# rhasspy/piper

Measured on AMD Instinct MI355X. Metric: audio samples/sec, higher is better.
Workload: dtype f32; 1 GPU; BASELINE configs[1]: medium VITS voice (22050 Hz), 1 utterance(s) x 128 phoneme ids per step per GPU, scales 0.667/1.0/0.8; step = inferSeconds span: host ids in (pe_upload) + pe_run, engine draws both noise sites + int16 PCM to host (pe_fetch); parallelism=utterance-parallel x1, one process per GPU, RCCL weight broadcast

## Files before the change

piper_amd/csrc/engine.h:

```cpp
#pragma once
#include <cstdint>
#include <deque>
#include <list>
#include <map>
#include <string>
#include <unordered_map>
#include <vector>

#include "pe_rt.h"
#include "engine_buffers.h"
#include "kernels/params.h"
#include "policy.h"
#include "weights.h"

namespace pe {

struct PackedConv {
  float* wp = nullptr;
  float* wp16 = nullptr;
  float* wpb = nullptr;
  const float* wunscale = nullptr;
  float* wpg4 = nullptr;
  float* bias = nullptr;
  int rows = 0;
// ... 84 lines not shown
  int native_rate() const { return rs_native_ ? rs_native_ : arch_[A_SR]; }
  int output_rate() const { return rs_on_ ? rs_out_ : native_rate(); }
  int resample_half_width() const { return rs_on_ ? rs_K_ : 0; }
  int64_t out_samples(int64_t s) const { return rs_on_ ? (s * rs_L_ + rs_M_ - 1) / rs_M_ : s; }
  void debug_resample(const float* x, int batch, int64_t stride, const int32_t* vlen, const int64_t* n0, const int32_t* count,
                      const int64_t* origin, float* out, int64_t out_stride);

  void set_loudness(bool on, float target_lufs, float ceiling_db);
  bool loudness_on() const { return ld_on_; }
  float loudness_target() const { return ld_T_; }
  float loudness_ceiling_db() const { return ld_cdb_; }
  int last_loudness(float* lufs, float* scale, float* peak, int32_t* flags, int64_t capacity);
  static void loudness_filter(int fs, double coef[10]);
  void set_loudness_ceiling(int kind);
  int loudness_ceiling_kind() const { return ld_kind_; }
  static int true_peak_oversample(int fs) { return fs > 0 ? (192000 + fs - 1) / fs : 0; }
  int last_true_peak(float* t, int64_t capacity);
  static void true_peak_filter(int fs, int& Q, int& K, std::vector<double>& coef);
  void debug_true_peak(const float* x, int batch, int64_t stride, const int32_t* valid, int fs, float* t);
  void set_loudness_limiter(bool on, float window_ms);
  bool loudness_limiter_on() const { return lim_on_; }
  float loudness_limiter_ms() const { return lim_ms_; }
  int loudness_limiter_window() const { return output_rate() > 0 ? limiter_window_samples(output_rate(), lim_ms_) : 0; }
  int last_limiter(float* max_reduction, int32_t* shaped_samples, float* trim, int64_t capacity);
  static void limiter_window(int fs, float window_ms, int& W, std::vector<double>& coef);
  void debug_limiter(const float* x, int batch, int64_t stride, const int32_t* valid, int fs, const float* g, float ceiling_db,
                     int kind, float window_ms, float* env, int16_t* pcm);
  void debug_loudness(const float* x, int batch, int64_t stride, const int32_t* valid, int fs, float target, float ceiling_db,
                      float* lufs, float* scale, int32_t* flags);

  void set_stream_gain(int mode, float peak, int ramp_samples);
  int stream_gain_mode() const { return gain_mode_; }
  float stream_gain_peak() const { return gain_peak_; }
  int stream_gain_ramp() const { return gain_ramp_; }
  int stream_last_gains(float* gain, float* peak, int64_t capacity);

  struct StreamChunk {
    int batch = 0;
    const int64_t* sample_offsets = nullptr;
    const int16_t* pcm = nullptr;
    const float* audio = nullptr;
    const int32_t* frames_done = nullptr;
  };
  const std::vector<int32_t>& stream_begin_batch(const int64_t* ids, const int64_t* offsets, int B, const float* scales,
                                                 const int64_t* sids, const NoiseIn* noise, const TimingIn* timing = nullptr,
                                                 const SeedsIn* seeds = nullptr, const BlendIn* blend = nullptr);
  void stream_next_batch(int chunk_frames, bool want_audio, StreamChunk& out);

  int stream_pool_open(int slots, int max_frames);
  void stream_pool_join(const int64_t* ids, const int64_t* offsets, int n, const float* scales, const int64_t* sids,
                        const NoiseIn* noise, int32_t* slot_of, int32_t* total_frames, const TimingIn* timing = nullptr,
                        const SeedsIn* seeds = nullptr, const BlendIn* blend = nullptr);
  void stream_pool_next(int chunk_frames, const int32_t* per_slot, bool want_audio, StreamChunk& out);
  void stream_pool_leave(int slot);
  void stream_pool_close();
  int stream_pool_state(int32_t* frames, int32_t* frames_done, int32_t* live) const;
  void stream_pool_require() const;

  int batch() const { return B_; }
  const std::vector<int64_t>& sample_offsets() { finish_run(); return sample_off_; }
  const float* audio_host() const { return h_audio_.get(); }
  const int16_t* pcm_host() const { return pcm_zc_live_ ? h_pcm_zc_.get() : h_pcm_.get(); }
  const std::vector<int32_t>& durations_host();
  const std::vector<int32_t>& frames_host() { finish_run(); return frames_h_; }
  void debug_tensor(const std::string& name, int b, std::vector<float>& out, int* rows, int* cols);
  void debug_randn(int site, uint64_t call, int64_t row, int64_t n, float* out);
  uint64_t rng_call() const { return call_; }
  long run_launches() const { return run_launches_; }
  long speculation_runs() const { return spec_runs_; }
  long speculation_misses() const { return spec_misses_; }
  const int* xcc_pattern(int* period) const { if (period) *period = xcd_period_; return xcc_of_; }

  void set_seed(uint64_t s) { seed_ = s; }
  uint64_t seed() const { return seed_; }
  void set_use_graphs(bool on) { use_graphs_ = on; }
  void set_profile(int level);
  const std::vector<ProfileRow>& profile();
  void reset_profile();
  hipStream_t stream() const { return stream_; }
  const int32_t* arch() const { return arch_; }
  int sample_rate() const { return arch_[A_SR]; }
  int hop() const { return hop_; }
  size_t weight_bytes() const { return weight_bytes_; }

 private:
  LaunchPolicy pol_;
  void init(const WeightSet& ws);
  float* dev_copy(const std::vector<float>& v);
  float* dev_alloc(size_t nfloats, const float* src);
  char* arena_ = nullptr; size_t arena_bytes_ = 0, arena_off_ = 0;
  bool arena_owned_ = false, skeleton_ = false;
  float* dev_tensor(const WeightSet& ws, const std::string& name);
  PackedConv pack_conv(const WeightSet& ws, const std::string& wname, const std::string& bname, int dil,
                       int padl_override, bool gate, int in_rev, int out_rev);
  PackedConv pack_qkv(const WeightSet& ws, const std::string& prefix, float** out16 = nullptr);
  PackedConv pack_convT(const WeightSet& ws, const std::string& prefix, int stride);
  PackedConv pack_matrix(const std::vector<float>& W, int rows, int Cin, int ntaps,
                         const std::vector<float>* bias, int nbias, int dil, int padl, bool gate, int split);
  DdsW load_dds(const WeightSet& ws, const std::string& prefix);
  enum Fill { FILL_NONE, FILL_ZERO, FILL_POISON, FILL_POISON_OR_ZERO };
  template <class Buf>
  void side_alloc(Buf& b, size_t n, bool idle, Fill fill, const char* what = nullptr, size_t what_bytes = 0);
  void ensure_stage_a(int B, int Tmax);
  void ensure_stage_b(int Fmax, int batch = 0);

  struct View { float* p; long bs; int cs; };
  struct ConvOpt {
    float in_slope = 1.f; int act = 0; View res{nullptr, 0, 0}; View out2{nullptr, 0, 0}; int mode = 0; float alpha = 1.f;
    const float* bias2 = nullptr; int bias2_bs = 0;
  };
  void conv(const PackedConv& pc, View x, View out, const int* lens, int len_mul, int Lmax, int epi, const ConvOpt& o);
  void conv(const PackedConv& pc, View x, View out, const int* lens, int len_mul, int Lmax, int epi) { conv(pc, x, out, lens, len_mul, Lmax, epi, ConvOpt()); }
  struct ConvPlan plan_conv(const PackedConv& pc, int Lmax, int epi, bool stage_tiled) const;
  bool grouping_ = false;
  bool stage_tiled_ = false;
  bool group_tiled_ = false;
  int group_cfg_ = 0;
  std::vector<struct ConvP> group_;
  double group_flops_ = 0, group_bytes_ = 0;
  int group_ncols_ = 0;
  void group_begin(bool tiled = false);
  void group_end();
  bool can_group_sum() const;
  void group_end_sum(View out, const float* bias_sum, float alpha);
  void layer_norm(View in, View out, const float* g, const float* b, int C, const int* lens, int Lmax);
  struct DdsOpt {
    const float* pre_z = nullptr; long pre_z_bs = 0; const float* pre_w = nullptr; const float* pre_b = nullptr;
    const float* z_scale = nullptr;
    const float* post_w16 = nullptr; const float* post_bias = nullptr; int post_rows = 0;
    View post_out{nullptr, 0, 0};
    const float* zin = nullptr; long zin_bs = 0; int z_cs = 0, c0 = 0, c1 = 1; float* zout = nullptr; long zout_bs = 0;
  };
  void dds(const DdsW& d, View in, View out, View tmp, const DdsOpt* opt = nullptr);
  double dds_bytes(const struct DdsP& p) const;
  double cols_ids_ = 0, cols_frames_ = 0;
  void dds_params(const DdsW& d, View in, View out, View tmp, const DdsOpt* opt, std::vector<struct DdsP>& list);
  float* pack16(const std::vector<float>& W, int rows, int K);
  float* pack4(const std::vector<float>& W, int rows, int K);
  std::unordered_map<const float*, const float*> w4_of_;
  const float* pack_ffn1(const WeightSet& ws, const std::string& wname);
  const float* pack_ffn2(const WeightSet& ws, const std::string& wname);
  DevBuf<float> ffn_parts_;
  bool stage_a_ffn_fused() const;
  float* stage_a_enc_out() const;
  const float* w4_of(const float* w16) const { auto it = w4_of_.find(w16); return it == w4_of_.end() ? nullptr : it->second; }
  float* dp_proj16_ = nullptr;
  float* dp_pre16_ = nullptr;
  float* projpre4_ = nullptr; float* projpre_bias_ = nullptr; int projpre_split_ = 0;
  void colchain(const struct ColP& p, int B, int Lmax, double flops);
  bool conv1x1_col4(const float* w16, const float* bias, int rows, View in, View out, const int* lens, int B, int Lmax,
                    double flops, const float* bias2 = nullptr, long bias2_bs = 0, const float* w4direct = nullptr, int kin = 192,
                    long max_cols = 0);
  const float* pack4_conv_pad192(const WeightSet& ws, const std::string& wname, int in_rev, int out_rev);
  struct LnSecond { const float* w4 = nullptr; int split = 0; View out2{nullptr, 0, 0}; const float* bias2 = nullptr; long bias2_bs = 0; };
  void lngemm(View y, const float* g, const float* b, View x, const float* w16, const float* bias, int rows, View out,
              int T, double flops, const float* parts = nullptr, int nparts = 0, const float* pbias = nullptr,
              const LnSecond* second = nullptr);
  bool proj_pre_stacked() const;
  float* pack16_conv(const WeightSet& ws, const std::string& wname, int in_rev, int out_rev);
  int xcc_of_[64] = {0};
  int xcd_period_ = 0;
  void probe_xcds();
  static size_t col4_smem() { return ((size_t)4 * 196 + 4 * 192 * 4 + 32 + 64 * 4) * sizeof(float); }
  void issue_stage_a();
  void issue_stage_b();
  void issue_flow();
  void issue_window();
  void issue_decoder(const float* zsrc, const int* lens, int Fmax, double fsum, bool zero_absmax, bool with_pcm16 = true,
                     const float* cond = nullptr, int cond_bs = 0);
  void run_stage(char which, const std::string& key);
  void dispatch_stage(char which);
  void drop_graphs();
  bool finish_run();
  void finish_stage_b_sizes();
  bool spec_pending_ = false;
  int spec_fg_ = 0;
  int spec_fg_force_ = 0;
  float last_ratio_ = 0.f, spec_margin_ = 1.10f;
  long spec_misses_ = 0, spec_runs_ = 0;
  int spec_hit_streak_ = 0, spec_recent_misses_ = 0, spec_recent_runs_ = 0, spec_cooldown_ = 0;
  int* d_framesc_ = nullptr;
  const int* lens_b_ = nullptr;
  void prof_begin();
  void prof_end(int row, double flops);

  int32_t arch_[ARCH_INTS];
  int device_ = 0;
  hipStream_t stream_ = nullptr;
  int H_, C_, FC_, nh_, dk_, nlayers_, ksz_, window_, hop_, U_;
  std::vector<void*> owned_;
  size_t weight_bytes_ = 0;

  float* emb_ = nullptr;
  float* emb_g_ = nullptr;
  struct EncLayer {
    PackedConv qkv, o, f1, f2;
    float* o16 = nullptr;
    float* qkv16 = nullptr;
    const float *f1p = nullptr, *f2p = nullptr;
    float *relk, *relv, *g1, *b1, *g2, *b2;
  };
  std::vector<EncLayer> enc_;
  PackedConv enc_proj_;
  float* enc_proj16_ = nullptr;
  PackedConv dp_pre_, dp_proj_;
  DdsW dp_dds_;
  struct CFlow {
    float *pre_w, *pre_b;
    DdsW dds;
    PackedConv proj;
    float* proj16 = nullptr;
  };
  std::vector<CFlow> cflows_;
  float ea_m0_ = 0, ea_es0_ = 1;
  float *ea_dev_m_ = nullptr, *ea_dev_logs_ = nullptr;
 public:
  void arena_ready();
 private:
  struct Rcl {
    PackedConv pre, post;
    float *pre16 = nullptr, *post16 = nullptr;
    const float* pre4pad = nullptr;
    std::vector<PackedConv> in, rs;
    std::vector<const float*> rs4;
    int in_off, out_off;
  };
  std::vector<Rcl> rcls_;
  PackedConv dec_pre_;
  struct UpStage {
    PackedConv up;
    int rate, ch;
    std::vector<std::vector<PackedConv>> rb;
    float* last_bias_sum = nullptr;
    struct HostConv { std::vector<float> w; int co = 0, ci = 0, k = 0, dil = 1; const float* bias = nullptr; };
    std::vector<std::vector<HostConv>> rb_host;
    void* mrf_phases = nullptr; float* mrf_w = nullptr;
    float* mrf_wsplit = nullptr; float* mrf_unscale = nullptr; int mrf_wsplit_floats = 0;
    int mrf_wfloats = 0, mrf_cp = 0, mrf_hx = 0;
    std::vector<struct MrfPhase> mrf_ph;
    bool mrf_ok = false, mrf_rb1 = false;
  };
  struct MrfGeo { int ou = 0, N = 0, cu_lo = 0, cu_hi = 0, nleft = 0, nhalo = 0; };
  bool mrf_geo(const UpStage& st, int len_mul, bool tail, MrfGeo& best) const;
  void build_mrf(UpStage& st);
  void mrf(const UpStage& st, View x, View out, const int* lens, int len_mul, int Lmax, bool tail = false);
  enum StageForm { STAGE_FUSED, STAGE_GROUP_SPLITK, STAGE_GROUP_TILED, STAGE_CHAIN };
  struct StageSchedule { StageForm form; bool tiled; };
  StageSchedule stage_schedule(const UpStage& st, int Lmax, double fsum, bool buffers_fit) const;
  bool matrix_bf3_ = false, pack_bf3_now_ = false;
  int matrix_sm_ = 0;
  static bool env_bf3();
 public:
  bool matrix_bf3() const { return matrix_bf3_; }
  int matrix_split_mode() const { return matrix_bf3_ ? matrix_sm_ : -1; }
 private:
  std::vector<UpStage> ups_;
  float* post_w_ = nullptr;
  int post_cin_ = 0;
  struct CondW { float* w; float* b; int rows; };
  CondW cond_dp_{nullptr, nullptr, 0}, cond_dec_{nullptr, nullptr, 0};
  std::vector<CondW> cond_wn_;
  int gin_ = 0, nspk_ = 1;

  int B_ = 0, Tmax_ = 0, Ts_ = 0, Fmax_ = 0, Fs_ = 0, Tg_ = 0, Fg_ = 0;
  bool use_graphs_ = true;
  struct GraphEntry { std::string key; void* exec; long launches; };
  std::list<GraphEntry> graphs_;
  std::unordered_map<std::string, std::list<GraphEntry>::iterator> graph_of_;
  long graph_captures_ = 0;
 public:
  long graph_captures() const { return graph_captures_; }
  size_t graphs_cached() const { return graphs_.size(); }
  static int id_bucket(int T);
  static int frame_bucket(int F);
  void warmup(int max_batch, int max_ids, float frames_per_id, const float* scales, const int64_t* sample, int64_t n_sample);
 private:
  long run_launches_ = 0;
  unsigned long long* d_rng_ = nullptr;
  float scales_[3] = {0.667f, 1.0f, 0.8f};
  std::vector<float> spec_rel_;
  float spec_rel(int b) const { return (size_t)b < spec_rel_.size() ? spec_rel_[b] : 1.f; }
  bool have_noise_w_ = false, have_noise_z_ = false;
  bool drew_w_ = false;
  bool plan_on_ = false, plan_skip_ = false;
  int* d_plan_ = nullptr; float* plan_w_ = nullptr;
  PinBuf<int> h_plan_;
  static bool check_timing(const TimingIn& t, const int64_t* offsets, int B);
  void plan_params(PlanP& pp, const DurP& dp) const;
  std::string stage_a_key(int B) const;
  bool fold_dur_ = false;
  DurP fold_dp_{};
  std::vector<int64_t> id_off_;
  std::vector<int32_t> tlens_h_, frames_h_, dur_h_;
  std::vector<int64_t> sample_off_;
  uint64_t seed_ = 1234, call_ = 0;
  const float* h_noise_z_ = nullptr;
  int64_t h_noise_z_stride_ = 0;

  size_t capA_B_ = 0, capA_T_ = 0, capB_B_ = 0, capB_F_ = 0;
  bool capB_exact_ = false;
  size_t ws_budget_ = 0;
  size_t ws_budget();
  DevBuf<char> wsA_, wsB_;
  int *d_ids_ = nullptr, *d_tlens_ = nullptr, *d_sids_ = nullptr, *d_dur_ = nullptr, *d_cum_ = nullptr,
      *d_frames_ = nullptr;
  float* d_scales_ = nullptr;
  static size_t in_scale_slots(size_t Bc) { return (3 * Bc + 3) & ~(size_t)3; }
  static size_t in_seed_bytes(size_t Bc) { return (12 * Bc + 15) & ~(size_t)15; }
  static size_t in_head_bytes(size_t Bc) { return 32 + in_seed_bytes(Bc); }
  unsigned long long* d_keys_ = nullptr; int* d_use_ = nullptr;
  bool seeded_ = false;
  const char* seed_key() const { return seeded_ ? "|s" : ""; }
  char* d_in_ = nullptr; PinBuf<char> h_in_; size_t in_bytes_ = 0;
  size_t in_blend_bytes(size_t Bc) const { return nspk_ > 1 ? (Bc * (68 + 4 * (size_t)gin_) + 255) & ~(size_t)255 : 0; }
  char* h_in() const { return h_in_.get() + in_blend_bytes(capA_B_); }
  char* d_blend_ = nullptr;
  float* g_tab_ = nullptr; int* g_rows_ = nullptr;
  bool blended_ = false;
  const char* blend_key() const { return blended_ ? "|g" : ""; }
  BlendP blend_params(const char* area, size_t Bc) const;
  bool ids_zc_ = false;
  unsigned long long upload_serial_ = 0;
  float* att_s_ = nullptr;
  size_t attn_smem(int T, bool global_scores) const;
  bool attn_scores_global(int T) const;
  float* vQ_ = nullptr;
  float* kT_ = nullptr;
  bool kt_on_ = false, kt_valid_ = false;
  float *x_ = nullptr, *y_ = nullptr, *qkv_ = nullptr, *att_ = nullptr, *ffh_ = nullptr, *stats_ = nullptr,
        *xg_ = nullptr, *dh_ = nullptr, *dy_ = nullptr, *dy2_ = nullptr, *hproj_ = nullptr, *z2_ = nullptr,
        *logw_ = nullptr, *noise_w_ = nullptr, *cond_ = nullptr;
  int cond_bs_ = 0;
  std::vector<int> cond_off_wn_;
  int cond_off_dp_ = 0, cond_off_dec_ = 0;
  float *zp_ = nullptr, *fh_ = nullptr, *facts_ = nullptr, *fskip_ = nullptr, *noise_z_ = nullptr;
  float* hb_[5] = {nullptr, nullptr, nullptr, nullptr, nullptr};
  hipStream_t ls_ = nullptr;
  DevBuf<float> side_[9];
  size_t side_floats_ = 0;
  float* zwin_ = nullptr;
  int* d_win_ = nullptr;
  int halo_frames_ = 0, s_frames_ = 0, s_pos_ = 0, s_wg_ = 0;
  bool s_active_ = false;
  std::vector<int16_t> s_pcm_;
  struct ChunkRows {
    char stage;
    int cap = 0;
    PinBuf<int> host; DevBuf<int> dev;
    PinBuf<int> gctl; DevBuf<int> gdev;
    std::vector<char> gfirst;
    std::vector<int32_t> pos;
    std::vector<int64_t> off;
    PinBuf<int16_t> pcm; PinBuf<float> audio;
    int wg = 0;
    const float* src = nullptr; long src_bs = 0; int src_cs = 0;
    const float* cond = nullptr; int cond_bs = 0;
  };
  void rows_free(ChunkRows& r);
  bool rows_next(ChunkRows& r, const int32_t* frames, const int32_t* live, int chunk, const int32_t* per_row, int clamp,
                 bool want_audio, StreamChunk& out);
  void issue_window_rows(const ChunkRows& r);
  bool sb_active_ = false;
  ChunkRows batch_rows_{'V'};
  void ensure_stream_batch(int B);
  int gain_mode_ = GAIN_CHUNK, gain_ramp_ = 0;
  float gain_peak_ = 0.f;
  float s_gain_r_ = 0.01f; bool s_gain_first_ = true;
  void gain_blocks_alloc(ChunkRows& r, int cap);
  void gain_prepare(int* ctl, int cap, const std::vector<char>& first, int n);
  void gain_collect(const int* ctl, int cap, int n, std::vector<char>& first, const int64_t* off, const unsigned* peaks);
  void gain_report_idle(const int* ctl, int cap, int n);
  std::vector<float> lg_gain_, lg_peak_;
  std::vector<char> lg_got_;
  int lg_n_ = -1;
  const unsigned* lg_dev_peaks_ = nullptr;
  bool lg_lazy_ = false;
  void stream_front(int B, int max_frames);
// ... 105 lines not shown
```

piper_amd/csrc/engine_issue.cpp:

```cpp
#include "engine_internal.h"

namespace pe {

bool Engine::stage_a_ffn_fused() const {
  double tsum = 0;
  for (int b = 0; b < B_; ++b) tsum += tlens_h_[b];
  const bool chain_q = pol_.chain16(tsum, false, H_, 96);
  bool f = pol_.ffn && chain_q && pol_.chain4((long)B_ * Tg_) && ffn_parts_ && (long)B_ * rup(Tg_, 4) <= LaunchPolicy::ffn_max_cols &&
           FC_ % 48 == 0 && FC_ / 48 <= 16 && w4_of(enc_proj16_);
  for (auto& e : enc_) f = f && e.f1p && e.f2p && w4_of(e.qkv16);
  return f;
}
bool Engine::proj_pre_stacked() const {
  double tsum = 0;
  for (int b = 0; b < B_; ++b) tsum += tlens_h_[b];
  return pol_.stack_pre && projpre4_ && projpre_split_ == enc_proj_.rows && dp_pre_.rows == 192 && H_ == 192 &&
         pol_.chain16(tsum, false, H_, 96) && pol_.chain4((long)B_ * Tg_);
}
float* Engine::stage_a_enc_out() const { return (stage_a_ffn_fused() && (enc_.size() & 1)) ? y_ : x_; }

void Engine::issue_stage_a() {
  const int B = B_, Ts = Ts_, T = Tg_;
  const long bsH = (long)H_ * Ts;
  auto V = [&](float* p, int ch) { return View{p, (long)ch * Ts, Ts}; };
// ... 134 lines not shown
    } else {
      conv(e.o, att, y, d_tlens_, 1, T, EPI_RESADD, {.res = x});
    }
    if (!chain_o) layer_norm(y, x, e.g1, e.b1, H_, d_tlens_, T);
    }
    if (ffn_fused) {
      FfnP fp{};
      fp.xcd = pol_.xcd_ffn ? xcd_period_ : 0;
      const int Tp = rup(T, 4);
      fp.x = x.p; fp.x_bs = x.bs; fp.x_cs = x.cs;
      fp.w1p = e.f1p; fp.b1 = e.f1.bias; fp.w2p = e.f2p;
      fp.parts = ffn_parts_.get(); fp.nslices = nsl; fp.p_bs = (long)nsl * H_ * Tp;
      fp.lens = d_tlens_;
      const int khf = kbegin(prof_level_ >= 2 ? krow("ffn_kernel") : 0, 2.0 * tsum * (e.f1.macs_per_col + e.f2.macs_per_col),
                             4.0 * (tsum * (1.0 + nsl) * H_ + e.f1.macs_per_col + e.f2.macs_per_col));
      const size_t smemf = ((size_t)192 * 48 + 4 * 48 * 16 + 48 * 48) * sizeof(float);
      launch::ffn(dim3((T + 11) / 12, nsl, B), smemf, stream_, fp);
      kend(khf);
      pend_bias = e.f2.bias;
    } else {
      conv(e.f1, x, ffh, d_tlens_, 1, T, EPI_STORE, {.act = ACT_RELU});
      conv(e.f2, ffh, y, d_tlens_, 1, T, EPI_RESADD, {.res = x});
    }
    if (chain_q) { pg = e.g2; pb = e.b2; }
    else layer_norm(y, x, e.g2, e.b2, H_, d_tlens_, T);
    fl += 2.0 * tsum * (e.qkv.macs_per_col + e.o.macs_per_col + e.f1.macs_per_col + e.f2.macs_per_col);
    for (int b = 0; b < B; ++b) fl += 2.0 * 2.0 * (double)tlens_h_[b] * tlens_h_[b] * H_;
  }
  const bool stacked = pg && proj_pre_stacked();
  LnSecond sec;
  if (stacked) {
    sec.w4 = projpre4_; sec.split = projpre_split_; sec.out2 = dy;
    sec.bias2 = cb_dp; sec.bias2_bs = cond_bs_;
  }
  const float* pj_bias = stacked ? projpre_bias_ : enc_proj_.bias;
  const int pj_rows = stacked ? projpre_split_ + dp_pre_.rows : enc_proj_.rows;
  const double pj_flops = 2.0 * tsum * (enc_proj_.macs_per_col + (stacked ? dp_pre_.macs_per_col : 0));
  if (pg && pend_bias) {
    lngemm(x, pg, pb, y, enc_proj16_, pj_bias, pj_rows, stats, T, pj_flops, ffn_parts_.get(), nsl, pend_bias, stacked ? &sec : nullptr);
    std::swap(x, y);
  } else if (pg) lngemm(y, pg, pb, x, enc_proj16_, pj_bias, pj_rows, stats, T, pj_flops, nullptr, 0, nullptr, stacked ? &sec : nullptr);
  else conv(enc_proj_, x, stats, d_tlens_, 1, T, EPI_STORE);
  if (x.p != stage_a_enc_out()) throw std::runtime_error("internal: encoder output buffer bookkeeping");
  fl += 2.0 * tsum * enc_proj_.macs_per_col;
  prof_end(0, fl);

  prof_begin();
  fl = 0;
  if (plan_skip_) {
    DurP dp{};
    dp.scales = d_scales_; dp.lens = d_tlens_; dp.dur = d_dur_; dp.cum = d_cum_; dp.d_bs = Ts; dp.frames = d_frames_;
    dp.frames_host = h_frames_.get(); dp.frames_clamped = d_framesc_; dp.frame_cap = std::max(Fs_, 1);
    PlanP pp{};
    plan_params(pp, dp);
    PE_LAUNCH_KB("duration_plan_kernel", 4.0 * 4.0 * tsum, launch::duration_plan(dim3(B), stream_, pp));
    prof_end(1, fl);
    return;
  }
  if (!stacked &&
      !(chain_q && dp_pre16_ && conv1x1_col4(dp_pre16_, dp_pre_.bias, dp_pre_.rows, x, dy, d_tlens_, B, T, 2.0 * tsum * dp_pre_.macs_per_col,
                                             cb_dp, cond_bs_)))
    conv(dp_pre_, x, dy, d_tlens_, 1, T, EPI_STORE, {.bias2 = cb_dp, .bias2_bs = cond_bs_});
  if (pol_.fuse_dp) {
    DdsOpt o;
    o.post_w16 = dp_proj16_; o.post_bias = dp_proj_.bias; o.post_rows = dp_proj_.rows; o.post_out = xg;
    dds(dp_dds_, dy, dh, dy2, &o);
  } else {
    dds(dp_dds_, dy, dh, dy2);
    conv(dp_proj_, dh, xg, d_tlens_, 1, T, EPI_STORE);
  }
  fl += 2.0 * tsum * (2 + arch_[A_DDSLAYERS]) * dp_pre_.macs_per_col;
  if (!have_noise_w_ && !drew_w_)
    PE_LAUNCH_KB("randn_kernel", 4.0 * 2.0 * tsum, launch::randn(stream_, noise_w_, (long)B * 2, T, (long)Ts, 0L, d_rng_, 0,
                                                               seeded_ ? d_keys_ : nullptr, d_use_, 2));
  if (!pol_.fuse_dp) {
    const long n = (long)B * 2 * Ts;
    PE_LAUNCH_K("scale_kernel", launch::scale(dim3((unsigned)((n + 255) / 256)), stream_, noise_w_, z2_, n, d_scales_ + 2, (long)2 * Ts));
  }
  int flips = 0;
  for (size_t fi = 0; fi < cflows_.size(); ++fi) {
    auto& cf = cflows_[fi];
    ++flips;
    const int c0 = (flips & 1) ? 1 : 0;
    const int c1 = 1 - c0;
    if (pol_.fuse_dp) {
      const float* zin = fi == 0 ? noise_w_ : z2_;
      DdsOpt o;
      o.pre_z = zin + (long)c0 * Ts; o.pre_z_bs = (long)2 * Ts; o.pre_w = cf.pre_w; o.pre_b = cf.pre_b;
      o.z_scale = fi == 0 ? d_scales_ + 2 : nullptr;
      o.post_w16 = cf.proj16; o.post_bias = cf.proj.bias; o.post_rows = cf.proj.rows;
      o.zin = zin; o.zin_bs = (long)2 * Ts; o.z_cs = Ts; o.c0 = c0; o.c1 = c1; o.zout = z2_; o.zout_bs = (long)2 * Ts;
      dds(cf.dds, xg, dh, dy2, &o);
    } else {
      PE_LAUNCH_K("cf_pre_kernel", launch::cf_pre(dim3((T + 63) / 64, H_, B), stream_, z2_ + (long)c0 * Ts, (long)2 * Ts, cf.pre_w, cf.pre_b, xg_, (long)H_ * Ts, Ts, dy_, (long)H_ * Ts, Ts, d_tlens_, H_));
      dds(cf.dds, dy, dh, dy2);
      conv(cf.proj, dh, hproj, d_tlens_, 1, T, EPI_STORE);
      PE_LAUNCH_K("spline_inverse_kernel", launch::spline_inverse(dim3((T + 63) / 64, B), stream_, hproj_, (long)32 * Ts, Ts, z2_ + (long)c1 * Ts, (long)2 * Ts, d_tlens_, 1.0f / std::sqrt((float)H_)));
    }
    fl += 2.0 * tsum * (arch_[A_DDSLAYERS] * dp_pre_.macs_per_col + cf.proj.macs_per_col);
  }
  ++flips;
  {
    const int c0 = (flips & 1) ? 1 : 0;
    DurP dp{};
    dp.z0 = z2_ + (long)c0 * Ts; dp.z_bs = (long)2 * Ts; dp.m0 = ea_m0_; dp.es0 = ea_es0_; dp.scales = d_scales_;
    dp.lens = d_tlens_; dp.dur = d_dur_; dp.cum = d_cum_; dp.d_bs = Ts; dp.frames = d_frames_; dp.logw_out = logw_;
    dp.frames_host = h_frames_.get(); dp.frames_clamped = d_framesc_; dp.frame_cap = std::max(Fs_, 1);
    fold_dp_ = dp;
    if (plan_on_) {
      PlanP pp{};
      plan_params(pp, dp);
      PE_LAUNCH_KB("duration_plan_kernel", 4.0 * 6.0 * tsum, launch::duration_plan(dim3(B), stream_, pp));
    } else if (!fold_dur_) PE_LAUNCH_KB("duration_kernel", 4.0 * 4.0 * tsum, launch::duration(dim3(B), stream_, dp));
  }
  prof_end(1, fl);
}

void Engine::issue_flow() {
  const int B = B_, Ts = Ts_, Fmax = Fg_, Fs = Fs_;
  double fsum = 0;
  for (int b = 0; b < B; ++b) fsum += frames_h_[b];
  cols_frames_ = fsum;
  double fl = 0;

  prof_begin();
  if (have_noise_z_) {
    if (h_noise_z_stride_ < Fmax_) throw std::runtime_error("noise_z stride shorter than the frame count");
    for (int b = 0; b < B; ++b)
      for (int c = 0; c < C_; ++c)
        PE_HIP(hipMemcpyAsync(noise_z_ + ((size_t)b * C_ + c) * Fs,
                              h_noise_z_ + ((size_t)b * C_ + c) * h_noise_z_stride_,
                              frames_h_[b] * sizeof(float), hipMemcpyHostToDevice, stream_));
  }
  {
    RegP rp{};
    rp.stats = stats_; rp.s_bs = (long)2 * C_ * Ts; rp.s_cs = Ts;
    rp.cum = d_cum_; rp.d_bs = Ts; rp.tlens = d_tlens_; rp.frames = lens_b_;
    rp.noise = noise_z_; rp.n_bs = (long)C_ * Fs; rp.n_cs = Fs;
    rp.scales = d_scales_;
    rp.out = zp_; rp.o_bs = (long)C_ * Fs; rp.o_cs = Fs; rp.C = C_;
    rp.absmax = absmax_;
    rp.rng = d_rng_; rp.gen = have_noise_z_ ? 0 : 1;
    if (seeded_) { rp.keys = d_keys_; rp.use = d_use_; }
    rp.fold = fold_dur_ ? 1 : 0;
    if (fold_dur_) rp.dur = fold_dp_;
    PE_LAUNCH_KB("regulate_kernel", 4.0 * (2.0 * C_ * cols_ids_ + 3.0 * C_ * fsum), launch::regulate(dim3((Fmax + 255) / 256, (C_ + 3) / 4, B), stream_, rp));
    if (zp_keep_)
      PE_HIP(hipMemcpyAsync(zp_keep_, zp_, (size_t)B * C_ * Fs * sizeof(float), hipMemcpyDeviceToDevice, stream_));
  }
  auto VF = [&](float* p, int ch) { return View{p, (long)ch * Fs, Fs}; };
  const View fh = VF(fh_, H_), facts = VF(facts_, H_), fskip = VF(fskip_, H_);
  const int half = C_ / 2;
  const bool chain = pol_.chain16(fsum, true, H_, half);
  for (size_t ri = 0; ri < rcls_.size(); ++ri) {
    Rcl& r = rcls_[ri];
    const View x0{zp_ + (long)r.in_off * Fs, (long)C_ * Fs, Fs};
    const View x1{zp_ + (long)r.out_off * Fs, (long)C_ * Fs, Fs};
    if (!(chain && ri > 0)) {
      if (!(chain && r.pre4pad && conv1x1_col4(nullptr, r.pre.bias, r.pre.rows, x0, fh, lens_b_, B, Fmax, 2.0 * fsum * r.pre.macs_per_col,
                                               nullptr, 0, r.pre4pad, half, LaunchPolicy::col4_max_frames)))
        conv(r.pre, x0, fh, lens_b_, 1, Fmax, EPI_STORE);
    }
    const int nl = (int)r.in.size();
    const bool rs_front = chain && nl >= 1 && r.rs4[nl - 1] && r.rs[nl - 1].rows == H_ && H_ == 192 && half == 96 &&
                          pol_.chain_rs_front((long)B * Fmax) && w4_of(r.post16) &&
                          (ri + 1 >= rcls_.size() || (rcls_[ri + 1].pre.rows <= 192 && w4_of(rcls_[ri + 1].pre16)));
    for (int i = 0; i < nl; ++i) {
      const float* b2 = nspk_ > 1 ? cond_ + cond_off_wn_[ri] + (long)i * 2 * H_ : nullptr;
      conv(r.in[i], fh, facts, lens_b_, 1, Fmax, EPI_GATE, {.bias2 = b2, .bias2_bs = cond_bs_});
      if (rs_front && i == nl - 1) {
        fl += 2.0 * fsum * (r.in[i].macs_per_col + r.rs[i].macs_per_col);
        continue;
      }
      if (r.rs4[i] && pol_.chain4_frames((long)B * Fmax) && H_ == 192 && r.rs[i].rows <= 2 * H_) {
        ColP cp{};
        cp.in1 = facts.p; cp.in1_bs = facts.bs; cp.in1_cs = facts.cs; cp.K1 = H_;
        cp.w1 = r.rs4[i]; cp.b1 = r.rs[i].bias; cp.rows1 = r.rs[i].rows;
        cp.mode = 2; cp.first = i == 0 ? 1 : 0;
        cp.xcd = xcd_period_;
        cp.x1 = fh.p; cp.x1_bs = fh.bs; cp.x1_cs = fh.cs;
        cp.out = fskip.p; cp.out_bs = fskip.bs; cp.out_cs = fskip.cs;
        cp.lens = lens_b_;
        const int kh4 = kbegin(prof_level_ >= 2 ? krow("colchain4_kernel<false>") : 0, 2.0 * fsum * r.rs[i].macs_per_col,
                               4.0 * (fsum * (H_ + 2.0 * cp.rows1) + (double)cp.rows1 * H_));
        launch::colchain4(dim3((Fmax + 3) / 4, B, (cp.rows1 + 191) / 192), col4_smem(), stream_, cp);
        kend(kh4);
      } else {
        conv(r.rs[i], facts, fh, lens_b_, 1, Fmax, EPI_WNRS, {.out2 = fskip, .mode = i == 0 ? 1 : 0});
      }
      fl += 2.0 * fsum * (r.in[i].macs_per_col + r.rs[i].macs_per_col);
    }
    if (chain) {
      ColP cp{};
      cp.in1 = fskip.p; cp.in1_bs = fskip.bs; cp.in1_cs = fskip.cs; cp.K1 = H_;
      cp.w1 = r.post16; cp.b1 = r.post.bias; cp.rows1 = half;
      cp.mode = 1;
      cp.x1 = x1.p; cp.x1_bs = x1.bs; cp.x1_cs = x1.cs;
      if (ri + 1 < rcls_.size()) {
        const Rcl& nx = rcls_[ri + 1];
        if (nx.in_off != r.out_off) throw std::runtime_error("coupling layers do not alternate halves");
        cp.w2 = nx.pre16; cp.b2 = nx.pre.bias; cp.rows2 = H_;
        cp.out2 = fh.p; cp.o2_bs = fh.bs; cp.o2_cs = fh.cs;
      }
      cp.lens = lens_b_;
      if (rs_front) {
        cp.in0 = facts.p; cp.in0_bs = facts.bs; cp.in0_cs = facts.cs;
        cp.w0 = r.rs4[nl - 1]; cp.b0 = r.rs[nl - 1].bias; cp.first = nl == 1 ? 1 : 0;
      }
      colchain(cp, B, Fmax, 2.0 * fsum * (r.post.macs_per_col + (cp.w2 ? rcls_[ri + 1].pre.macs_per_col : 0) +
                                          (rs_front ? r.rs[nl - 1].macs_per_col : 0)));
    } else {
      conv(r.post, fskip, x1, lens_b_, 1, Fmax, EPI_SUBFROM);
    }
    fl += 2.0 * fsum * (r.pre.macs_per_col + r.post.macs_per_col);
  }
  prof_end(2, fl);

}

void Engine::issue_stage_b() {
  issue_flow();
  double fsum = 0;
  for (int b = 0; b < B_; ++b) fsum += frames_h_[b];
  issue_decoder(zp_, lens_b_, Fg_, fsum, false);
}

void Engine::issue_window() {
  PE_LAUNCH_K("window_copy_kernel", launch::window_copy(dim3((s_wg_ + 63) / 64, C_), stream_, zp_, Fs_, d_win_, zwin_, Fs_, C_));
  issue_decoder(zwin_, d_win_ + 1, s_wg_, (double)s_wg_, true);
  if (rs_on_) issue_resample(1, audio_, Ss_, rs_host_.get(), nullptr, out_samples((long)s_wg_ * hop_) + 1, (double)s_wg_ * hop_);
}

void Engine::issue_window_rows(const ChunkRows& r) {
  const int B = (int)r.pos.size(), cap = r.cap, wg = r.wg;
  int *const dst = r.dev.get(), *const gctl = r.gctl.get(), *const gdev = r.gdev.get();
  struct Restore { int& b; int b0; ~Restore() { b = b0; } } restore{B_, B_};
  B_ = B;
  const int gm = gain_mode_;
  if (gm != GAIN_CHUNK && (!gctl || !gdev || B > cap)) throw std::runtime_error("stream gain blocks are not sized for this call");
  PE_LAUNCH_KB("window_gather_kernel", 8.0 * B * C_ * wg,
               launch::window_gather(dim3((wg + 63) / 64, C_, B), stream_, r.src, r.src_bs, r.src_cs, r.host.get(), dst, cap,
                                     noise_z_, (long)C_ * Fs_, Fs_, wg));
  std::vector<int32_t> win((size_t)B, wg);
  frames_h_.swap(win);
  try {
    issue_decoder(noise_z_, dst + sb_o_len(cap), wg, (double)B * wg, true, false, r.cond, r.cond_bs);
  } catch (...) {
    frames_h_.swap(win);
    throw;
  }
  frames_h_.swap(win);
  if (rs_on_) {
    const long max_out = out_samples((long)wg * hop_) + 1;
    issue_resample(B, audio_, Ss_, rs_host_.get(), nullptr, max_out, (double)B * wg * hop_);
    const int rsteps = std::max(1, (int)((max_out + CHUNK_SPB - 1) / CHUNK_SPB));
    if (gm != GAIN_CHUNK) {
      PE_LAUNCH_K("stream_gain_kernel", launch::stream_gain(stream_, gctl, gdev, cap, B, gm, dst, hop_, rs_dev_.get(), rs_cap_, So_));
      PE_LAUNCH_KB("chunk_pcm_rs_gain_kernel", 10.0 * B * (double)max_out,
                   launch::chunk_pcm_rs_gain(dim3(rsteps, B), stream_, raudio_.get(), So_, rs_dev_.get(), rs_cap_, dst, cap, gdev));
      return;
    }
    PE_LAUNCH_KB("chunk_pcm_rs_kernel", 10.0 * B * (double)max_out,
                 launch::chunk_pcm_rs(dim3(rsteps, B), stream_, raudio_.get(), So_, rs_dev_.get(), rs_cap_, dst, cap));
    return;
  }
  const int steps = std::max(1, (int)(((long)wg * hop_ + CHUNK_SPB - 1) / CHUNK_SPB));
  if (gm != GAIN_FIXED)
    PE_LAUNCH_KB("chunk_peak_kernel", 4.0 * B * wg * hop_, launch::chunk_peak(dim3(steps, B), stream_, audio_, Ss_, dst, cap, hop_));
  if (gm != GAIN_CHUNK) {
    PE_LAUNCH_K("stream_gain_kernel", launch::stream_gain(stream_, gctl, gdev, cap, B, gm, dst, hop_, nullptr, 0, 0));
    PE_LAUNCH_KB("chunk_pcm_gain_kernel", 10.0 * B * wg * hop_,
                 launch::chunk_pcm_gain(dim3(steps, B), stream_, audio_, Ss_, dst, cap, hop_, gdev));
    return;
  }
  PE_LAUNCH_KB("chunk_pcm_kernel", 10.0 * B * wg * hop_, launch::chunk_pcm(dim3(steps, B), stream_, audio_, Ss_, dst, cap, hop_));
}

void Engine::issue_decoder(const float* zsrc, const int* lens, int Fmax, double fsum, bool zero_absmax, bool with_pcm16,
                           const float* cond, int cond_bs) {
  const int B = B_, Fs = Fs_;
  const float* cb_dec = nspk_ > 1 ? (cond ? cond : cond_ + cond_off_dec_) : nullptr;
  const int cb_dec_bs = cond ? cond_bs : cond_bs_;
  double fl = 0;
  bool tail_done = false;
  if (zero_absmax) PE_HIP(hipMemsetAsync(absmax_, 0, B * sizeof(unsigned), stream_));
  prof_begin();
  fl = 0;
  {
    View cur{hb_[0], (long)U_ * Fs, Fs};
    conv(dec_pre_, View{const_cast<float*>(zsrc), (long)C_ * Fs, Fs}, cur, lens, 1, Fmax, EPI_STORE, {.bias2 = cb_dec, .bias2_bs = cb_dec_bs});
    fl += 2.0 * fsum * dec_pre_.macs_per_col;
    int mult = 1;
    int cur_buf = 0;
    const int nk = arch_[A_NRB];
    const float inv_nk = 1.0f / (float)nk;
    for (auto& st : ups_) {
      int ids[5], n = 0;
      for (int i = 0; i < 5 && n < 4; ++i)
        if (i != cur_buf) ids[n++] = i;
      const int Lin = mult;
      mult *= st.rate;
      const long Ls = (long)Fs * mult;
      auto VS = [&](int bi) { return View{hb_[bi], (long)st.ch * Ls, (int)Ls}; };
      const View u = VS(ids[0]), ta = VS(ids[1]), tb = VS(ids[2]), tc = VS(ids[3]);
      const int Lmax = Fmax * mult;
      const StageSchedule sched = stage_schedule(st, Lmax, fsum, (size_t)B * st.ch * Ls <= side_floats_);
      const bool fuse = sched.form == STAGE_FUSED, grp_t = sched.form == STAGE_GROUP_TILED;
      const bool tail = fuse && pol_.mrf_tail && &st == &ups_.back() && st.mrf_cp == 32 && st.ch == post_cin_ && mult == hop_;
      conv(st.up, cur, u, lens, Lin, Fmax * Lin, EPI_CONVT, {.in_slope = 0.1f});
      fl += 2.0 * fsum * Lin * st.up.macs_per_col;
      struct Scope { bool& f; ~Scope() { f = false; } } scope{stage_tiled_};
      stage_tiled_ = sched.tiled;
      const View xs{hb_[cur_buf], (long)st.ch * Ls, (int)Ls};
      auto chain = [&](int j, const View (&t)[3], View dst, int accmode) {
        auto& cv = st.rb[j];
        const int last_epi = EPI_ACCUM;
        View xin = u;
        if (arch_[A_RESBLOCK] == 1) {
          const int np = (int)cv.size() / 2;
          for (int d = 0; d < np; ++d) {
            conv(cv[2 * d], xin, t[0], lens, mult, Lmax, EPI_STORE, {.in_slope = 0.1f});
            if (d < np - 1) {
              const View nxt = (d & 1) ? t[2] : t[1];
              conv(cv[2 * d + 1], t[0], nxt, lens, mult, Lmax, EPI_RESADD, {.in_slope = 0.1f, .res = xin});
              xin = nxt;
            } else {
              conv(cv[2 * d + 1], t[0], dst, lens, mult, Lmax, last_epi, {.in_slope = 0.1f, .res = xin, .mode = accmode, .alpha = inv_nk});
            }
            fl += 2.0 * fsum * mult * (cv[2 * d].macs_per_col + cv[2 * d + 1].macs_per_col);
          }
        } else {
          const int nc = (int)cv.size();
          for (int d = 0; d < nc; ++d) {
            if (d < nc - 1) {
              const View nxt = (d & 1) ? t[2] : t[1];
              conv(cv[d], xin, nxt, lens, mult, Lmax, EPI_RESADD, {.in_slope = 0.1f, .res = xin});
              xin = nxt;
            } else {
              conv(cv[d], xin, dst, lens, mult, Lmax, last_epi, {.in_slope = 0.1f, .res = xin, .mode = accmode, .alpha = inv_nk});
            }
            fl += 2.0 * fsum * mult * cv[d].macs_per_col;
          }
        }
      };
      if (fuse) {
        mrf(st, u, xs, lens, mult, Lmax, tail);
        for (auto& cv : st.rb)
          for (auto& c : cv) fl += 2.0 * fsum * mult * c.macs_per_col;
        if (tail) {
          tail_done = true;
          fl += 2.0 * fsum * hop_ * post_cin_ * POST_K;
// ... 67 lines not shown
```

piper_amd/csrc/engine_launch.cpp:

```cpp
#include "engine_internal.h"

namespace pe {


static int tile_cfg_of(int cfg) { return cfg == CFG_C ? CFG_C : CFG_S; }
static int slab_halo(int xhalo) { return xhalo <= 64 ? 64 : 128; }
static size_t tile_smem(int nbuf, int BN, int halo) { return (size_t)nbuf * KC * ((BN + halo + 63) / 64 * 64) * sizeof(float); }
static size_t splitk_smem(int nw, int MT, int xw) { return std::max<size_t>((size_t)nw * KC * xw, (size_t)nw * MT * 16 * 64) * sizeof(float); }

ConvPlan Engine::plan_conv(const PackedConv& pc, int Lmax, int epi, bool stage_tiled) const {
  ConvPlan pl;
  const bool convt = epi == EPI_CONVT;
  const int ncols = pl.ncols = convt ? Lmax + 1 : Lmax;
  const int xhalo = (pc.ntaps - 1) * pc.dil, units = pc.nchunks * pc.ntaps;
  pl.blocks = tile_workgroups(CFG_BM[pc.cfg], CFG_BN[pc.cfg], ncols, pc.mtiles, B_);
  pl.halo = slab_halo(xhalo);
  const bool to_splitk = !stage_tiled && pol_.splitk(pl.blocks, xhalo, pc.Cin);
  const bool direct = pol_.one_tap_direct(pc.gate, convt, pc.ntaps, pc.Cin);
  pl.group_splitk = !stage_tiled && !convt && pol_.groupable(pc.gate, pc.up != 0, pl.blocks, xhalo, pc.Cin);
  pl.group_tiled = !pc.gate && pc.up == 0 && !convt && !to_splitk && !(matrix_bf3_ && pc.wpb) && !direct && xhalo <= 128;
  pl.group_cfg = tile_cfg_of(pc.cfg);
  if (to_splitk && epi == EPI_GATE &&
      pol_.gate_12col(pc.gate, pc.wpg4 != nullptr && pc.Cin == 192, pc.ntaps, pc.dil, tile_workgroups(32, 12, ncols, pc.split / 32, B_))) {
    pl.form = CONV_GATE12;
// ... 92 lines not shown
    if (cv.size() != st.rb[0].size()) grp = grp_t = false;
    for (auto& c : cv) {
      const ConvPlan pl = plan_conv(c, Lmax, EPI_STORE, tiled);
      grp = grp && pl.group_splitk;
      grp_t = grp_t && pl.group_tiled && pl.group_cfg == tc;
    }
  }
  return {grp ? STAGE_GROUP_SPLITK : (grp_t ? STAGE_GROUP_TILED : STAGE_CHAIN), tiled};
}

void Engine::group_begin(bool tiled) {
  grouping_ = true;
  group_tiled_ = tiled;
  group_cfg_ = -1;
  group_.clear();
  group_flops_ = group_bytes_ = 0;
}
void Engine::group_end() {
  grouping_ = false;
  if (group_.empty()) return;
  if (group_tiled_) {
    group_tiled_ = false;
    std::stable_sort(group_.begin(), group_.end(), [](const ConvP& a, const ConvP& b) { return a.ntaps > b.ntaps; });
    ConvG g{};
    int n = 0, rows = 0, xhalo = 0;
    for (const ConvP& c : group_) {
      g.c[n++] = c;
      rows = std::max(rows, c.rows);
      xhalo = std::max(xhalo, c.xhalo);
    }
    g.n = n;
    g.B = B_;
    const int cfg = group_cfg_, BM = CFG_BM[cfg], BN = CFG_BN[cfg];
    const int HALO = slab_halo(xhalo);
    const dim3 grid((group_ncols_ + BN - 1) / BN, (rows + BM - 1) / BM, n * B_);
    int kh = -1;
    if (prof_level_ >= 2) {
      char nm[96];
      snprintf(nm, sizeof(nm), "conv_mfma_group_kernel<%s,%d>", cfg == CFG_C ? "1,4,1,1,16" : "2,2,1,1,16", HALO);
      kh = kbegin(krow(std::string(nm)), group_flops_, group_bytes_);
    }
    launch::conv_tile_group(cfg, HALO, grid, tile_smem(2, BN, HALO), ls_, g);
    kend(kh);
    group_.clear();
    return;
  }
  constexpr int NW = 4;
  std::stable_sort(group_.begin(), group_.end(), [](const ConvP& a, const ConvP& b) { return a.ntaps > b.ntaps; });
  for (int wide = 0; wide < 2; ++wide) {
    ConvG g{};
    int n = 0, mt = 0;
    for (const ConvP& c : group_)
      if ((c.xhalo > 32) == (wide == 1)) {
        g.c[n++] = c;
        mt = std::max(mt, (c.rows + 31) / 32);
      }
    if (!n) continue;
    g.n = n;
    g.B = B_;
    const dim3 grid((group_ncols_ + 31) / 32, mt, n * B_);
    const double share = (double)n / (double)group_.size();
    const int kh = kbegin(prof_level_ >= 2 ? krow(wide ? "conv_splitk_group_kernel<4,2,128>" : "conv_splitk_group_kernel<4,2,64>") : 0,
                          group_flops_ * share, group_bytes_ * share);
    launch::conv_group(wide != 0, grid, splitk_smem(NW, 1, wide ? 128 : 64), ls_, g);
    kend(kh);
  }
  group_.clear();
}

bool Engine::can_group_sum() const {
  if (group_.size() < 2 || group_.size() > 3) return false;
  const ConvP& a = group_[0];
  for (const ConvP& c : group_)
    if (c.rows != a.rows || c.Cin != a.Cin || c.nchunks != a.nchunks || c.x_bs != a.x_bs || c.x_cs != a.x_cs ||
        c.r_bs != a.r_bs || c.r_cs != a.r_cs || c.in_slope != a.in_slope || c.epi != EPI_RESADD || c.xhalo > 96)
      return false;
  return true;
}
void Engine::group_end_sum(View out, const float* bias_sum, float alpha) {
  grouping_ = false;
  if (!can_group_sum()) throw std::runtime_error("internal: convs do not fit a K-concatenated launch");
  ConvP q = group_[0];
  q.nseg = (int)group_.size();
  for (int i = 0; i < q.nseg; ++i) {
    q.seg_x[i] = group_[i].x; q.seg_wp[i] = group_[i].wp;
    q.seg_ntaps[i] = group_[i].ntaps; q.seg_dil[i] = group_[i].dil; q.seg_padl[i] = group_[i].padl;
  }
  q.res2 = group_[1].res;
  q.res3 = q.nseg > 2 ? group_[2].res : nullptr;
  q.bias = bias_sum;
  q.out = out.p; q.o_bs = out.bs; q.o_cs = out.cs;
  q.epi = EPI_ACCUM; q.mode = 3; q.alpha = alpha;
  q.tgroups = 1;
  const dim3 grid((group_ncols_ + 31) / 32, (q.rows + 31) / 32, B_);
  const int kh = kbegin(prof_level_ >= 2 ? krow("conv_splitk_sum_kernel<4,2>") : 0, group_flops_, group_bytes_);
  launch::conv_group_sum(grid, splitk_smem(4, 1, 128), ls_, q);
  kend(kh);
  group_.clear();
}

static void conv_cost(const PackedConv& pc, int epi, int mode, double cols, double& flops, double& bytes) {
  const bool rd_res = epi == EPI_RESADD || epi == EPI_ACCUM;
  const bool rd_old = epi == EPI_SUBFROM || epi == EPI_WNRS || (epi == EPI_ACCUM && (mode == 1 || mode == 2));
  const double out_rows = epi == EPI_GATE ? pc.split : pc.rows;
  flops = 2.0 * pc.macs_per_col * cols;
  bytes = 4.0 * (cols * (pc.Cin + out_rows * (1 + (rd_res ? 1 : 0) + (rd_old ? 1 : 0))) + (double)pc.rows * pc.Cin * pc.ntaps);
}

void Engine::conv(const PackedConv& pc, View x, View out, const int* lens, int len_mul, int Lmax, int epi, const ConvOpt& o) {
  if ((epi == EPI_GATE) != pc.gate) throw std::runtime_error("internal: gate epilogue/packing mismatch");
  ConvP p;
  p.x = x.p; p.x_bs = x.bs; p.x_cs = x.cs;
  p.wp = pc.wp; p.wp16 = pc.wp16; p.wpb = pc.wpb; p.wunscale = pc.wunscale; p.wpg4 = nullptr; p.bias = pc.bias;
  p.bias2 = o.bias2; p.bias2_bs = o.bias2_bs;
  p.out = out.p; p.o_bs = out.bs; p.o_cs = out.cs;
  p.res = o.res.p; p.r_bs = o.res.bs; p.r_cs = o.res.cs;
  p.out2 = o.out2.p; p.o2_bs = o.out2.bs; p.o2_cs = o.out2.cs;
  p.lens = lens; p.len_mul = len_mul;
  p.Cin = pc.Cin; p.rows = pc.rows; p.nchunks = pc.nchunks;
  p.ntaps = pc.ntaps; p.dil = pc.dil; p.padl = pc.padl; p.xhalo = (pc.ntaps - 1) * pc.dil;
  p.in_slope = o.in_slope; p.epi = epi; p.act = o.act; p.mode = o.mode; p.alpha = o.alpha;
  p.split = (epi == EPI_GATE) ? pc.split : (epi == EPI_WNRS ? (pc.rows > H_ ? H_ : 0) : 0);
  p.up = pc.up; p.padT = pc.padT; p.up_magic = pc.up ? (unsigned)((0x100000000ULL + pc.up - 1) / pc.up) : 0u;
  p.up_vec = 0; p.tpb = 1; p.tgroups = 1;
  double kflops = 0, kbytes = 0;
  if (prof_level_ >= 2) {
    const std::vector<int32_t>& lh = (lens == d_tlens_) ? tlens_h_ : frames_h_;
    double cols = 0;
    for (int b = 0; b < B_; ++b) cols += (double)lh[b] * len_mul;
    conv_cost(pc, epi, o.mode, cols, kflops, kbytes);
  }
  const ConvPlan pl = plan_conv(pc, Lmax, epi, stage_tiled_);
  if (grouping_) {
    if (!(group_tiled_ ? pl.group_tiled : pl.group_splitk) || group_.size() >= 3 ||
        (!group_.empty() && (group_ncols_ != pl.ncols || (group_tiled_ && group_cfg_ != pl.group_cfg))))
      throw std::runtime_error(group_tiled_ ? "internal: conv does not fit a grouped tiled launch" : "internal: conv does not fit a grouped launch");
    group_cfg_ = pl.group_cfg;
    group_.push_back(p);
    group_ncols_ = pl.ncols;
    group_flops_ += kflops; group_bytes_ += kbytes;
    return;
  }
  p.up_vec = pl.up_vec; p.tpb = pl.tpb; p.tgroups = pl.tgroups;
  if (pl.form == CONV_GATE12) p.wpg4 = pc.wpg4;
  const int kh = prof_level_ >= 2 ? kbegin(krow(conv_row_name(pl, pc, matrix_sm_, pol_.prof_sites != 0, epi, len_mul)), kflops, kbytes) : -1;
  switch (pl.form) {
    case CONV_GATE12: launch::gate4(pl.grid, pl.smem, ls_, p); break;
    case CONV_SPLITK: launch::conv_splitk(pc.gate, pl.nw, pl.grid, pl.smem, ls_, p); break;
    case CONV_SPLITK16: launch::conv_splitk16(pc.gate, pl.grid, pl.smem, ls_, p, pl.half); break;
    case CONV_SPLIT: launch::conv_bf3(matrix_sm_, pl.cfg, pc.gate, pl.halo, pl.grid, pl.smem, ls_, p); break;
    case CONV_1X1: launch::conv1x1(pl.grid, ls_, p); break;
    case CONV_TILE: launch::conv_tile(pl.cfg, pc.gate, pl.halo, pl.grid, pl.smem, ls_, p); break;
  }
  kend(kh);
}

bool Engine::mrf_geo(const UpStage& st, int len_mul, bool tail, MrfGeo& best) const {
  const int CP = st.mrf_cp, NCG = CP == 32 ? 8 : 4, HU = CP == 32 ? 1 : 2;
  const int OUMAX = CP == 32 ? 4 : 3;
  const int hx = st.mrf_hx, hxa = rup(hx, 16);
  auto geo = [&](int ou, MrfGeo& g) {
    g.ou = ou; g.N = 16 * NCG * ou;
    if (hxa + g.N + hx > mrf_ws(CP, ou)) return false;
    g.cu_lo = (hxa - hx) / 16; g.cu_hi = (hxa + g.N + hx + 15) / 16;
    g.nleft = hxa / 16 - g.cu_lo; g.nhalo = g.cu_hi - g.cu_lo - g.N / 16;
    return g.nhalo <= NCG * HU;
  };
  best = MrfGeo{};
  double best_cost = 0;
  MrfGeo forced;
  const int force = (pol_.mrf_ou >= 1 && pol_.mrf_ou <= OUMAX && geo((int)pol_.mrf_ou, forced)) ? (int)pol_.mrf_ou : 0;
  for (int ou = 1; ou <= OUMAX; ++ou) {
    MrfGeo g;
    if ((force && ou != force) || !geo(ou, g)) continue;
    double wgs = 0;
    const int stride = tail ? g.N - (POST_K - 1) : g.N;
    for (int b = 0; b < B_; ++b) wgs += (double)(((long)frames_h_[b] * len_mul + stride - 1) / stride);
    double work = 0, taps = 0;
    for (auto& P : st.mrf_ph) {
      const int lo = (hxa - P.e) / 16, hi = (hxa + g.N + P.e + 15) / 16;
      work += (double)(hi - lo) * 16 * P.ntaps;
      taps += P.ntaps;
    }
    double cost = std::ceil(wgs / 256.0) * (work + 16.0 * taps);
    if (ou == 4) cost *= 1.06;
    if (!best.ou || cost < best_cost) { best = g; best_cost = cost; }
  }
  return best.ou != 0;
}

void Engine::mrf(const UpStage& st, View x, View out, const int* lens, int len_mul, int Lmax, bool tail) {
  const int CP = st.mrf_cp, HU = CP == 32 ? 1 : 2;
  const int hx = st.mrf_hx, hxa = rup(hx, 16);
  MrfGeo best;
  if (!mrf_geo(st, len_mul, tail, best)) throw std::runtime_error("internal: no mrf_kernel geometry for this stage");
  MrfP p{};
  p.x = x.p; p.x_bs = x.bs; p.x_cs = x.cs;
  p.out = out.p; p.o_bs = out.bs; p.o_cs = out.cs;
  p.lens = lens; p.len_mul = len_mul;
  p.phases = static_cast<const MrfPhase*>(st.mrf_phases); p.nphases = (int)st.mrf_ph.size();
  p.wstream = st.mrf_w; p.wfloats = st.mrf_wfloats;
  p.C = st.ch; p.N = best.N; p.wcols = hxa + best.N + hx; p.hxa = hxa; p.cu_lo = best.cu_lo; p.cu_hi = best.cu_hi;
  p.nleft = best.nleft; p.nhalo = best.nhalo;
  p.slope = 0.1f;
  p.alpha = 1.0f / (float)st.rb.size();
  p.stride = best.N; p.n0off = 0;
  p.post_w = nullptr; p.audio = nullptr; p.a_bs = 0; p.absmax = nullptr; p.post_slope = 0.01f;
  if (tail) {
    p.stride = best.N - (POST_K - 1); p.n0off = (POST_K - 1) / 2;
    p.post_w = post_w_; p.audio = audio_; p.a_bs = Ss_; p.absmax = absmax_;
  }
  double kflops = 0, kbytes = 0;
  if (prof_level_ >= 2) {
    double cols = 0;
    for (int b = 0; b < B_; ++b) cols += (double)frames_h_[b] * len_mul;
    double macs = 0;
    for (auto& cv : st.rb)
      for (auto& c : cv) macs += c.macs_per_col;
    kflops = 2.0 * macs * cols;
    kbytes = 8.0 * st.ch * cols + 4.0 * st.mrf_wfloats;
    if (tail) {
      kflops += 2.0 * cols * st.ch * POST_K;
      kbytes = 4.0 * (st.ch + 1) * cols + 4.0 * st.mrf_wfloats;
    }
  }
  dim3 grid((Lmax + p.stride - 1) / p.stride, B_);
  char nm[64];
  const bool split = matrix_bf3_ && pol_.mrf_split && st.mrf_wsplit != nullptr && matrix_sm_ < 2;
  if (split) {
    p.wstream = st.mrf_wsplit; p.wfloats = st.mrf_wsplit_floats; p.wunscale = st.mrf_unscale;
    snprintf(nm, sizeof(nm), "mrf_split_kernel<%d,%d,%d,%d>", matrix_sm_, CP, best.ou, HU);
  } else {
    snprintf(nm, sizeof(nm), "mrf_kernel<%d,%d,%d>", CP, best.ou, HU);
  }
  const int kh = prof_level_ >= 2 ? kbegin(krow(std::string(nm)), kflops, kbytes) : -1;
  if (split) launch::mrf_split(matrix_sm_, CP, best.ou, grid, ls_, p);
  else launch::mrf(CP, best.ou, grid, ls_, p);
  kend(kh);
}

size_t Engine::attn_smem(int T, bool global_scores) const {
  const int SP = rup(T, 64) + 1, VS = dk_ + 1 + (dk_ & 1);
  return ((global_scores ? 0 : (size_t)ATT_QB * SP) + (size_t)ATT_KCH * VS + (size_t)dk_ * ATT_QB +
          (size_t)2 * (2 * window_ + 1) * dk_ + 4 * ATT_QB * 16) * sizeof(float);
}
bool Engine::attn_scores_global(int T) const { return pol_.attn_long || attn_smem(T, false) > (size_t)160 * 1024; }

void Engine::layer_norm(View in, View out, const float* g, const float* b, int C, const int* lens, int Lmax) {
  LnP p;
  p.in = in.p; p.i_bs = in.bs; p.i_cs = in.cs;
  p.out = out.p; p.o_bs = out.bs; p.o_cs = out.cs;
  p.gamma = g; p.beta = b;
  p.lens = lens; p.C = C;
  if (C > LN_COLS * 32) throw std::runtime_error("LayerNorm over more than 256 channels is not supported");
  dim3 grid((Lmax + LN_COLS - 1) / LN_COLS, B_);
  const int kh = kbegin(prof_level_ >= 2 ? krow("ln_kernel") : 0, 0.0, 4.0 * 2.0 * C * (lens == d_tlens_ ? cols_ids_ : cols_frames_));
  launch::layer_norm(grid, stream_, p);
  kend(kh);
}

void Engine::dds_params(const DdsW& d, View in, View out, View tmp, const DdsOpt* opt, std::vector<DdsP>& list) {
  int dil = 1;
  const int n = (int)d.c1x1.size();
  View cur = in;
  for (int i = 0; i < n; ++i) {
    const View dst = ((n - 1 - i) & 1) ? tmp : out;
    if (dst.p == cur.p) throw std::runtime_error("internal: DDSConv buffer aliasing");
    DdsP p{};
    if (opt && i == 0 && opt->pre_z) {
      p.pre_z = opt->pre_z; p.pre_z_bs = opt->pre_z_bs; p.pre_w = opt->pre_w; p.pre_b = opt->pre_b;
    }
    p.z_scale = opt ? opt->z_scale : nullptr;
    if (opt && i == n - 1 && opt->post_w16) {
      p.post_w16 = opt->post_w16; p.post_w4 = w4_of(opt->post_w16); p.post_bias = opt->post_bias; p.post_rows = opt->post_rows;
      p.post_out = opt->post_out.p; p.po_bs = opt->post_out.bs; p.po_cs = opt->post_out.cs;
      p.zin = opt->zin; p.zin_bs = opt->zin_bs; p.z_cs = opt->z_cs; p.c0 = opt->c0; p.c1 = opt->c1;
      p.zout = opt->zout; p.zout_bs = opt->zout_bs;
      p.inv_sqrt_h = 1.0f / std::sqrt((float)H_);
    }
    p.x = cur.p; p.x_bs = cur.bs; p.x_cs = cur.cs;
    p.out = dst.p; p.o_bs = dst.bs; p.o_cs = dst.cs;
    p.dw_w = d.dw_w[i]; p.dw_b = d.dw_b[i]; p.dw_k = ksz_; p.dw_dil = dil;
    p.g1 = d.g1[i]; p.b1 = d.b1[i]; p.g2 = d.g2[i]; p.b2 = d.b2[i];
    p.bias = d.c1x1[i].bias;
    p.wp16 = d.w16[i];
    p.wp4 = w4_of(d.w16[i]);
    p.nchunks = d.c1x1[i].nchunks;
    p.lens = d_tlens_; p.H = H_;
    list.push_back(p);
    dil *= ksz_;
    cur = dst;
  }
}

double Engine::dds_bytes(const DdsP& p) const {
  return 4.0 * (cols_ids_ * (2.0 * H_ + p.post_rows) + (double)H_ * H_ + (double)p.post_rows * H_);
}

void Engine::dds(const DdsW& d, View in, View out, View tmp, const DdsOpt* opt) {
  std::vector<DdsP> list;
  dds_params(d, in, out, tmp, opt, list);
  bool four = H_ == 192 && ksz_ <= 3 && pol_.chain4((long)B_ * Tg_);
  for (const DdsP& p : list) four = four && p.wp4 && (!p.post_w16 || p.post_w4);
  for (const DdsP& p : list) {
    if (four) {
      const int kh4 = kbegin(prof_level_ >= 2 ? krow("dds_layer4_kernel") : 0, 0.0, dds_bytes(p));
// ... 168 lines not shown
```

piper_amd/csrc/engine_pack.cpp:

```cpp
#include "engine_internal.h"
#include <cmath>

namespace pe {


float* Engine::dev_alloc(size_t nfloats, const float* src) {
  arena_off_ = (arena_off_ + 255) / 256 * 256;
  const size_t bytes = std::max<size_t>(nfloats, 1) * sizeof(float);
  if (arena_off_ + bytes > arena_bytes_) throw std::runtime_error("internal: packed weights exceed the arena bound");
  float* d = reinterpret_cast<float*>(arena_ + arena_off_);
  arena_off_ += bytes;
  if (src && nfloats && !skeleton_) PE_HIP(hipMemcpy(d, src, nfloats * sizeof(float), hipMemcpyHostToDevice));
  weight_bytes_ += nfloats * sizeof(float);
  return d;
}
float* Engine::dev_copy(const std::vector<float>& v) { return dev_alloc(v.size(), v.data()); }

float* Engine::dev_tensor(const WeightSet& ws, const std::string& name) {
  const HostTensor& t = ws.get(name);
  return dev_alloc((size_t)t.numel(), t.data.empty() ? nullptr : t.data.data());
}

size_t Engine::arena_bound(const WeightSet& ws) {
  size_t n = 0;
// ... 159 lines not shown
  if (w.dims.size() != 3) throw std::runtime_error(wname + ": expected a rank-3 conv weight");
  const int Co = (int)w.dims[0], Ci = (int)w.dims[1], K = (int)w.dims[2];
  std::vector<float> W(skeleton_ ? 0 : (size_t)Co * Ci * K);
  if (!skeleton_) {
    if (w.data.size() != W.size()) throw std::runtime_error(wname + ": data size mismatch");
    for (int o = 0; o < Co; ++o)
      for (int i = 0; i < Ci; ++i)
        for (int k = 0; k < K; ++k) {
          const int so = out_rev ? Co - 1 - o : o, si = in_rev ? Ci - 1 - i : i;
          W[((size_t)o * Ci + i) * K + k] = w.data[((size_t)so * Ci + si) * K + k];
        }
  }
  std::vector<float> bias;
  bool has_b = !bname.empty() && ws.has(bname);
  if (has_b) {
    if (ws.get(bname).numel() != Co) throw std::runtime_error(bname + ": bias size mismatch");
    if (!skeleton_) {
      bias = ws.get(bname).data;
      if (out_rev) std::reverse(bias.begin(), bias.end());
    }
  }
  const int padl = padl_override >= 0 ? padl_override : (K - 1) * dil / 2;
  return pack_matrix(W, Co, Ci, K, has_b ? &bias : nullptr, Co, dil, padl, gate, gate ? Co / 2 : 0);
}

PackedConv Engine::pack_qkv(const WeightSet& ws, const std::string& prefix, float** out16) {
  std::vector<float> W, bias;
  int H = 0;
  for (const char* n : {"conv_q", "conv_k", "conv_v"}) {
    const HostTensor& w = ws.get(prefix + "." + n + ".weight");
    const HostTensor& b = ws.get(prefix + "." + n + ".bias");
    H = (int)w.dims[0];
    if (!skeleton_) {
      W.insert(W.end(), w.data.begin(), w.data.end());
      bias.insert(bias.end(), b.data.begin(), b.data.end());
    }
  }
  if (out16) *out16 = pack16(W, 3 * H, H);
  return pack_matrix(W, 3 * H, H, 1, &bias, 3 * H, 1, 0, false, 0);
}

PackedConv Engine::pack_convT(const WeightSet& ws, const std::string& prefix, int stride) {
  const HostTensor& w = ws.get(prefix + ".weight");
  const int Ci = (int)w.dims[0], Co = (int)w.dims[1], K = (int)w.dims[2];
  if (K != 2 * stride || ((K - stride) & 1))
    throw std::runtime_error(prefix + ": ConvTranspose1d with kernel != 2*stride is not supported");
  const int rows = Co * stride;
  std::vector<float> W(skeleton_ ? 0 : (size_t)rows * Ci * 2);
  for (int co = 0; co < (skeleton_ ? 0 : Co); ++co)
    for (int ph = 0; ph < stride; ++ph)
      for (int ci = 0; ci < Ci; ++ci) {
        const size_t row = (size_t)co * stride + ph;
        W[(row * Ci + ci) * 2 + 0] = w.data[((size_t)ci * Co + co) * K + ph + stride];
        W[(row * Ci + ci) * 2 + 1] = w.data[((size_t)ci * Co + co) * K + ph];
      }
  std::vector<float> bias = ws.get(prefix + ".bias").data;
  PackedConv pc = pack_matrix(W, rows, Ci, 2, &bias, Co, 1, 1, false, 0);
  pc.up = stride;
  pc.padT = (K - stride) / 2;
  return pc;
}

float* Engine::pack16(const std::vector<float>& W, int rows, int K) {
  const int Kp = rup(K, 32), nq = Kp / 16, ntile = (rows + 15) / 16;
  const size_t np = (size_t)ntile * nq * 256;
  std::vector<float> P(skeleton_ ? 0 : np, 0.f);
  for (int mt = 0; mt < (skeleton_ ? 0 : ntile); ++mt)
    for (int q = 0; q < nq; ++q)
      for (int lane = 0; lane < 64; ++lane)
        for (int jj = 0; jj < 4; ++jj) {
          const int row = mt * 16 + (lane & 15), ci = 4 * (4 * q + jj) + (lane >> 4);
          if (row < rows && ci < K) P[(((size_t)mt * nq + q) * 64 + lane) * 4 + jj] = W[(size_t)row * K + ci];
        }
  float* d16 = dev_alloc(np, skeleton_ ? nullptr : P.data());
  if (const float* d4 = pack4(W, rows, K)) w4_of_[d16] = d4;
  return d16;
}

float* Engine::pack4(const std::vector<float>& W, int rows, int K) {
  if (K != 192 && K != 96) return nullptr;
  const int nq = K / 4, ntile = (rows + 63) / 64;
  const size_t np = (size_t)ntile * nq * 256;
  std::vector<float> P(skeleton_ ? 0 : np, 0.f);
  for (int mt = 0; mt < (skeleton_ ? 0 : ntile); ++mt)
    for (int q = 0; q < nq; ++q)
      for (int lane = 0; lane < 64; ++lane)
        for (int jj = 0; jj < 4; ++jj) {
          const int row = mt * 64 + lane;
          if (row < rows) P[(((size_t)mt * nq + q) * 64 + lane) * 4 + jj] = W[(size_t)row * K + 4 * q + jj];
        }
  return dev_alloc(np, skeleton_ ? nullptr : P.data());
}

const float* Engine::pack_ffn1(const WeightSet& ws, const std::string& wname) {
  const HostTensor& w = ws.get(wname);
  if (w.dims.size() != 3 || w.dims[1] != 192 || w.dims[2] != 3 || w.dims[0] % 48 || w.dims[0] / 48 > 16) return nullptr;
  const int FC = (int)w.dims[0], S = FC / 48;
  const size_t np = (size_t)FC * 192 * 3;
  std::vector<float> P(skeleton_ ? 0 : np, 0.f);
  for (int s = 0; s < (skeleton_ ? 0 : S); ++s)
    for (int m = 0; m < 3; ++m)
      for (int wv = 0; wv < 4; ++wv)
        for (int tp = 0; tp < 3; ++tp)
          for (int q = 0; q < 3; ++q)
            for (int lane = 0; lane < 64; ++lane)
              for (int j = 0; j < 4; ++j) {
                const int row = 48 * s + 16 * m + (lane & 15), ch = 48 * wv + 4 * (4 * q + j) + (lane >> 4);
                P[(((((size_t)(s * 3 + m) * 4 + wv) * 3 + tp) * 3 + q) * 64 + lane) * 4 + j] = w.data[((size_t)row * 192 + ch) * 3 + tp];
              }
  return dev_alloc(np, skeleton_ ? nullptr : P.data());
}
const float* Engine::pack_ffn2(const WeightSet& ws, const std::string& wname) {
  const HostTensor& w = ws.get(wname);
  if (w.dims.size() != 3 || w.dims[0] != 192 || w.dims[2] != 3 || w.dims[1] % 48 || w.dims[1] / 48 > 16) return nullptr;
  const int FC = (int)w.dims[1], S = FC / 48;
  const size_t np = (size_t)FC * 192 * 3;
  std::vector<float> P(skeleton_ ? 0 : np, 0.f);
  for (int s = 0; s < (skeleton_ ? 0 : S); ++s)
    for (int rt = 0; rt < 12; ++rt)
      for (int tp = 0; tp < 3; ++tp)
        for (int q = 0; q < 3; ++q)
          for (int lane = 0; lane < 64; ++lane)
            for (int j = 0; j < 4; ++j) {
              const int row = 16 * rt + (lane & 15), hid = 48 * s + 4 * (4 * q + j) + (lane >> 4);
              P[((((size_t)(s * 12 + rt) * 3 + tp) * 3 + q) * 64 + lane) * 4 + j] = w.data[((size_t)row * FC + hid) * 3 + tp];
            }
  return dev_alloc(np, skeleton_ ? nullptr : P.data());
}

float* Engine::pack16_conv(const WeightSet& ws, const std::string& wname, int in_rev, int out_rev) {
  const HostTensor& w = ws.get(wname);
  if (w.dims.size() != 3 || w.dims[2] != 1) throw std::runtime_error(wname + ": expected a 1x1 conv weight");
  const int Co = (int)w.dims[0], Ci = (int)w.dims[1];
  std::vector<float> W(skeleton_ ? 0 : (size_t)Co * Ci);
  if (!skeleton_)
    for (int o = 0; o < Co; ++o)
      for (int i = 0; i < Ci; ++i)
        W[(size_t)o * Ci + i] = w.data[(size_t)(out_rev ? Co - 1 - o : o) * Ci + (in_rev ? Ci - 1 - i : i)];
  return pack16(W, Co, Ci);
}

const float* Engine::pack4_conv_pad192(const WeightSet& ws, const std::string& wname, int in_rev, int out_rev) {
  const HostTensor& w = ws.get(wname);
  if (w.dims.size() != 3 || w.dims[2] != 1 || w.dims[1] > 192) return nullptr;
  const int Co = (int)w.dims[0], Ci = (int)w.dims[1];
  std::vector<float> W(skeleton_ ? 0 : (size_t)Co * 192, 0.f);
  if (!skeleton_)
    for (int o = 0; o < Co; ++o)
      for (int i = 0; i < Ci; ++i)
        W[(size_t)o * 192 + i] = w.data[(size_t)(out_rev ? Co - 1 - o : o) * Ci + (in_rev ? Ci - 1 - i : i)];
  return pack4(W, Co, 192);
}

DdsW Engine::load_dds(const WeightSet& ws, const std::string& p) {
  DdsW d;
  for (int i = 0; i < arch_[A_DDSLAYERS]; ++i) {
    const std::string s = std::to_string(i);
    d.dw_w.push_back(dev_tensor(ws, p + ".convs_sep." + s + ".weight"));
    d.dw_b.push_back(dev_tensor(ws, p + ".convs_sep." + s + ".bias"));
    d.c1x1.push_back(pack_conv(ws, p + ".convs_1x1." + s + ".weight", p + ".convs_1x1." + s + ".bias", 1, -1,
                               false, 0, 0));
    {
      const HostTensor& w1 = ws.get(p + ".convs_1x1." + s + ".weight");
      d.w16.push_back(pack16(w1.data, (int)w1.dims[0], (int)w1.dims[1]));
    }
    d.g1.push_back(dev_tensor(ws, p + ".norms_1." + s + ".gamma"));
    d.b1.push_back(dev_tensor(ws, p + ".norms_1." + s + ".beta"));
    d.g2.push_back(dev_tensor(ws, p + ".norms_2." + s + ".gamma"));
    d.b2.push_back(dev_tensor(ws, p + ".norms_2." + s + ".beta"));
  }
  return d;
}

void Engine::init(const WeightSet& ws) {
  pol_.read_env();
  use_graphs_ = !pol_.no_graph;
  matrix_bf3_ = env_bf3();
  matrix_sm_ = std::max(0, LaunchPolicy::matrix_mode_env());
  memcpy(arch_, ws.arch, sizeof(arch_));
  PE_HIP(hipSetDevice(device_));
  PE_HIP(hipStreamCreateWithFlags(&stream_, hipStreamNonBlocking));
  ls_ = stream_;
  H_ = arch_[A_HIDDEN]; C_ = arch_[A_INTER]; FC_ = arch_[A_FILTER]; nh_ = arch_[A_NHEADS];
  nlayers_ = arch_[A_NLAYERS]; ksz_ = arch_[A_KSIZE]; window_ = arch_[A_WINDOW]; U_ = arch_[A_UPINIT];
  gin_ = arch_[A_GIN]; nspk_ = arch_[A_NSPK];
  if (H_ <= 0 || C_ <= 0 || nh_ <= 0 || H_ % nh_ || (C_ & 1)) throw std::runtime_error("bad architecture header");
  dk_ = H_ / nh_;
  if (dk_ > 128 || (dk_ & 1)) throw std::runtime_error("head dimension must be even and <= 128");
  if ((2 * window_ + 1) * dk_ > 1280 || window_ > 4)
    throw std::runtime_error("relative-attention window too wide (window <= 4, (2*window+1) * head dim <= 1280)");
  if (H_ % 32 || H_ > 256) throw std::runtime_error("hidden_channels must be a multiple of 32 and <= 256");
  if (ksz_ > 3 || !(ksz_ & 1)) throw std::runtime_error("kernel_size must be 1 or 3");
  hop_ = 1;
  for (int i = 0; i < arch_[A_NUPS]; ++i) hop_ *= arch_[A_UPR0 + i];

  emb_ = dev_tensor(ws, "enc_p.emb.weight");
  const int padl_ffn = (ksz_ - 1) / 2;
  for (int l = 0; l < nlayers_; ++l) {
    const std::string s = std::to_string(l), a = "enc_p.encoder.attn_layers." + s,
                      f = "enc_p.encoder.ffn_layers." + s;
    EncLayer e;
    e.qkv = pack_qkv(ws, a, &e.qkv16);
    e.o = pack_conv(ws, a + ".conv_o.weight", a + ".conv_o.bias", 1, -1, false, 0, 0);
    e.o16 = pack16_conv(ws, a + ".conv_o.weight", 0, 0);
    e.relk = dev_tensor(ws, a + ".emb_rel_k");
    e.relv = dev_tensor(ws, a + ".emb_rel_v");
    e.g1 = dev_tensor(ws, "enc_p.encoder.norm_layers_1." + s + ".gamma");
    e.b1 = dev_tensor(ws, "enc_p.encoder.norm_layers_1." + s + ".beta");
    e.f1 = pack_conv(ws, f + ".conv_1.weight", f + ".conv_1.bias", 1, padl_ffn, false, 0, 0);
    e.f2 = pack_conv(ws, f + ".conv_2.weight", f + ".conv_2.bias", 1, padl_ffn, false, 0, 0);
    if (H_ == 192 && ksz_ == 3 && padl_ffn == 1) {
      e.f1p = pack_ffn1(ws, f + ".conv_1.weight");
      e.f2p = pack_ffn2(ws, f + ".conv_2.weight");
    }
    e.g2 = dev_tensor(ws, "enc_p.encoder.norm_layers_2." + s + ".gamma");
    e.b2 = dev_tensor(ws, "enc_p.encoder.norm_layers_2." + s + ".beta");
    enc_.push_back(e);
  }
  enc_proj_ = pack_conv(ws, "enc_p.proj.weight", "enc_p.proj.bias", 1, -1, false, 0, 0);
  enc_proj16_ = pack16_conv(ws, "enc_p.proj.weight", 0, 0);

  dp_pre_ = pack_conv(ws, "dp.pre.weight", "dp.pre.bias", 1, -1, false, 0, 0);
  dp_pre16_ = (H_ == 192) ? pack16_conv(ws, "dp.pre.weight", 0, 0) : nullptr;
  projpre4_ = nullptr;
  projpre_bias_ = nullptr;
  projpre_split_ = 0;
  if (H_ == 192) {
    const HostTensor& wp = ws.get("enc_p.proj.weight");
    const HostTensor& wd = ws.get("dp.pre.weight");
    const HostTensor& bp = ws.get("enc_p.proj.bias");
    const HostTensor& bd = ws.get("dp.pre.bias");
    if (wp.dims.size() == 3 && wd.dims.size() == 3 && wp.dims[1] == 192 && wd.dims[1] == 192 && wp.dims[2] == 1 && wd.dims[2] == 1 &&
        wp.dims[0] % 192 == 0 && wd.dims[0] == 192) {
      const int rp = (int)wp.dims[0], rd = (int)wd.dims[0];
      std::vector<float> Wst(skeleton_ ? 0 : (size_t)(rp + rd) * 192), Bst(skeleton_ ? 0 : (size_t)(rp + rd));
      if (!skeleton_) {
        std::copy(wp.data.begin(), wp.data.begin() + (size_t)rp * 192, Wst.begin());
        std::copy(wd.data.begin(), wd.data.begin() + (size_t)rd * 192, Wst.begin() + (size_t)rp * 192);
        std::copy(bp.data.begin(), bp.data.begin() + rp, Bst.begin());
        std::copy(bd.data.begin(), bd.data.begin() + rd, Bst.begin() + rp);
      }
      projpre4_ = pack4(Wst, rp + rd, 192);
      projpre_bias_ = dev_alloc((size_t)(rp + rd), skeleton_ ? nullptr : Bst.data());
      projpre_split_ = rp;
    }
  }
  dp_dds_ = load_dds(ws, "dp.convs");
  dp_proj_ = pack_conv(ws, "dp.proj.weight", "dp.proj.bias", 1, -1, false, 0, 0);
  {
    const HostTensor& w = ws.get("dp.proj.weight");
    dp_proj16_ = pack16(w.data, (int)w.dims[0], (int)w.dims[1]);
  }
  for (int i = arch_[A_DPFLOWS] - 1; i >= 1; --i) {
    const std::string p = "dp.flows." + std::to_string(2 * i + 1);
    CFlow cf;
    cf.pre_w = dev_tensor(ws, p + ".pre.weight");
    cf.pre_b = dev_tensor(ws, p + ".pre.bias");
    cf.dds = load_dds(ws, p + ".convs");
    cf.proj = pack_conv(ws, p + ".proj.weight", p + ".proj.bias", 1, -1, false, 0, 0);
    if (cf.proj.rows != 3 * arch_[A_NBINS] - 1 || arch_[A_NBINS] != 10)
      throw std::runtime_error("spline with num_bins != 10 is not supported");
    {
      const HostTensor& w = ws.get(p + ".proj.weight");
      cf.proj16 = pack16(w.data, (int)w.dims[0], (int)w.dims[1]);
    }
    cflows_.push_back(cf);
  }
  {
    ea_dev_m_ = dev_tensor(ws, "dp.flows.0.m");
    ea_dev_logs_ = dev_tensor(ws, "dp.flows.0.logs");
    if (!skeleton_) {
      ea_m0_ = ws.get("dp.flows.0.m").data[0];
      ea_es0_ = std::exp(-ws.get("dp.flows.0.logs").data[0]);
    }
  }

  pack_bf3_now_ = matrix_bf3_;
  {
    const int nf = arch_[A_FLOWN], half = C_ / 2, wnl = arch_[A_WNLAYERS], wnk = arch_[A_WNK];
    int flips = 0;
    for (int f = nf - 1; f >= 0; --f) {
      ++flips;
      const bool odd = flips & 1;
      const std::string p = "flow.flows." + std::to_string(2 * f);
      Rcl r;
      r.in_off = odd ? half : 0;
      r.out_off = odd ? 0 : half;
      r.pre = pack_conv(ws, p + ".pre.weight", p + ".pre.bias", 1, -1, false, odd, 0);
      for (int i = 0; i < wnl; ++i) {
        const std::string s = std::to_string(i);
        r.in.push_back(pack_conv(ws, p + ".enc.in_layers." + s + ".weight", p + ".enc.in_layers." + s + ".bias",
                                 1, -1, true, 0, 0));
        r.rs.push_back(pack_conv(ws, p + ".enc.res_skip_layers." + s + ".weight",
                                 p + ".enc.res_skip_layers." + s + ".bias", 1, -1, false, 0, 0));
        {
          const HostTensor& wrs = ws.get(p + ".enc.res_skip_layers." + s + ".weight");
          r.rs4.push_back(wrs.dims.size() == 3 && wrs.dims[2] == 1 ? pack4(wrs.data, (int)wrs.dims[0], (int)wrs.dims[1]) : nullptr);
        }
        (void)wnk;
      }
      r.post = pack_conv(ws, p + ".post.weight", p + ".post.bias", 1, -1, false, 0, odd);
      r.pre16 = pack16_conv(ws, p + ".pre.weight", odd, 0);
      if (H_ == 192 && rcls_.empty()) r.pre4pad = pack4_conv_pad192(ws, p + ".pre.weight", odd, 0);
      r.post16 = pack16_conv(ws, p + ".post.weight", 0, odd);
      rcls_.push_back(r);
      if (gin_) {
        const HostTensor& cw = ws.get(p + ".enc.cond_layer.weight");
        cond_wn_.push_back(CondW{dev_tensor(ws, p + ".enc.cond_layer.weight"), dev_tensor(ws, p + ".enc.cond_layer.bias"),
                                 (int)cw.dims[0]});
      }
    }
    if (flips & 1) throw std::runtime_error("odd number of flow layers is not supported");
  }

  dec_pre_ = pack_conv(ws, "dec.conv_pre.weight", "dec.conv_pre.bias", 1, -1, false, 0, 0);
  {
    const int nk = arch_[A_NRB], nd = arch_[A_NDIL];
    int ch = U_;
    for (int i = 0; i < arch_[A_NUPS]; ++i) {
      UpStage st;
      st.rate = arch_[A_UPR0 + i];
      st.up = pack_convT(ws, "dec.ups." + std::to_string(i), st.rate);
      ch = U_ >> (i + 1);
      st.ch = ch;
      for (int j = 0; j < nk; ++j) {
        const std::string rb = "dec.resblocks." + std::to_string(i * nk + j);
        std::vector<PackedConv> cv;
        std::vector<UpStage::HostConv> hv;
        auto add = [&](const std::string& wn, const std::string& bn, int dil) {
          cv.push_back(pack_conv(ws, wn, bn, dil, -1, false, 0, 0));
          const HostTensor& w = ws.get(wn);
          UpStage::HostConv h;
          h.w = w.data; h.co = (int)w.dims[0]; h.ci = (int)w.dims[1]; h.k = (int)w.dims[2]; h.dil = dil;
          h.bias = cv.back().bias;
          hv.push_back(std::move(h));
        };
        for (int d = 0; d < nd; ++d) {
          const int dil = arch_[A_RBDIL0 + j * MAX_DIL + d];
          const std::string s = std::to_string(d);
          if (arch_[A_RESBLOCK] == 1) {
            add(rb + ".convs1." + s + ".weight", rb + ".convs1." + s + ".bias", dil);
            add(rb + ".convs2." + s + ".weight", rb + ".convs2." + s + ".bias", 1);
          } else {
            add(rb + ".convs." + s + ".weight", rb + ".convs." + s + ".bias", dil);
          }
        }
        st.rb.push_back(cv);
        st.rb_host.push_back(std::move(hv));
      }
      {
        std::vector<float> bs(skeleton_ ? 0 : (size_t)ch, 0.f);
        for (int j = 0; j < nk; ++j) {
          const std::string rb = "dec.resblocks." + std::to_string(i * nk + j);
          const std::string bn = rb + (arch_[A_RESBLOCK] == 1 ? ".convs2." : ".convs.") + std::to_string(nd - 1) + ".bias";
          if (!ws.has(bn) || ws.get(bn).numel() != ch) throw std::runtime_error(bn + ": bias size mismatch");
          if (!skeleton_)
            for (int c = 0; c < ch; ++c) bs[c] += ws.get(bn).data[c];
        }
        st.last_bias_sum = dev_alloc((size_t)ch, skeleton_ ? nullptr : bs.data());
      }
      build_mrf(st);
      st.rb_host.clear();
      ups_.push_back(st);
    }
    const HostTensor& pw = ws.get("dec.conv_post.weight");
    post_w_ = dev_tensor(ws, "dec.conv_post.weight");
    post_cin_ = (int)pw.dims[1];
    if ((int)pw.dims[0] != 1 || post_cin_ != ch || (int)pw.dims[2] != POST_K)
      throw std::runtime_error("dec.conv_post shape mismatch");
  }

  pack_bf3_now_ = false;
  if (nspk_ > 1) {
    if (!gin_) throw std::runtime_error("multi-speaker voice without gin_channels");
    emb_g_ = dev_tensor(ws, "emb_g.weight");
    const HostTensor& dw = ws.get("dp.cond.weight");
    cond_dp_ = CondW{dev_tensor(ws, "dp.cond.weight"), dev_tensor(ws, "dp.cond.bias"), (int)dw.dims[0]};
    const HostTensor& cw = ws.get("dec.cond.weight");
    cond_dec_ = CondW{dev_tensor(ws, "dec.cond.weight"), dev_tensor(ws, "dec.cond.bias"), (int)cw.dims[0]};
    cond_off_dp_ = 0;
    int off = cond_dp_.rows;
    for (auto& c : cond_wn_) { cond_off_wn_.push_back(off); off += c.rows; }
    cond_off_dec_ = off;
    off += cond_dec_.rows;
    cond_bs_ = off;
  }

  {
    long r = 3;
    const int nk = arch_[A_NRB], nd = arch_[A_NDIL];
    for (int i = (int)ups_.size() - 1; i >= 0; --i) {
      long widest = 0;
      for (int j = 0; j < nk; ++j) {
        const long hk = (arch_[A_RBK0 + j] - 1) / 2;
        long w = 0;
        for (int d = 0; d < nd; ++d) {
          w += hk * arch_[A_RBDIL0 + j * MAX_DIL + d];
          if (arch_[A_RESBLOCK] == 1) w += hk;
        }
        widest = std::max(widest, w);
      }
      r += widest;
      r = (r + ups_[i].rate - 1) / ups_[i].rate + 1;
    }
    halo_frames_ = (int)(r + 3);
  }
  launch::init_conv();
  launch::init_bf3();
  launch::init_front();
  launch::init_tail();
  probe_xcds();
  static const char* rows[] = {"text_encoder", "duration_predictor", "regulate+flow", "hifigan", "post+pcm"};
  for (auto n : rows) prof_.push_back(ProfileRow{n});
  PE_HIP(hipEventCreate(&ev0_));
  PE_HIP(hipEventCreate(&ev1_));
  h_frames_.grow(4096);
}

void Engine::build_mrf(UpStage& st) {
  const int ch = st.ch;
  if (!pol_.mrf_build(ch) || st.rb_host.empty()) return;
  const int CP = ch <= 32 ? 32 : 64, MS = CP / 16, NCH = CP / KC, STEPF = MS * 512;
  const bool rb1 = arch_[A_RESBLOCK] == 1;
  int hx = 0;
  for (auto& hv : st.rb_host) {
    int e = 0;
    for (auto& h : hv) e += h.dil * (h.k - 1) / 2;
    hx = std::max(hx, e);
  }
  const int hxa = rup(hx, 16);
  std::vector<MrfPhase> phases;
  std::vector<float> wstream;
  const bool split = matrix_bf3_ && matrix_sm_ < 2;
  std::vector<uint16_t> wsplit;
  std::vector<float> unscale;
  for (size_t j = 0; j < st.rb_host.size(); ++j) {
    auto& hv = st.rb_host[j];
    const int n = (int)hv.size();
    if (n == 0 || (rb1 && (n & 1))) return;
    int e = 0;
    for (auto& h : hv) {
      if (!(h.k & 1) || h.ci != ch || h.co != ch) return;
      e += h.dil * (h.k - 1) / 2;
    }
    for (int i = 0; i < n; ++i) {
      const auto& h = hv[i];
      e -= h.dil * (h.k - 1) / 2;
      MrfPhase P{};
      P.bias = h.bias; P.ntaps = h.k; P.dil = h.dil; P.e = e;
      const bool last = i == n - 1;
      if (rb1) {
        if (!(i & 1)) { P.src = 0; P.dst = 1; P.flags = 0; }
        else { P.src = 1; P.dst = last ? -1 : 0; P.flags = MRF_RES | MRF_KEEP; }
      } else {
        P.src = i == 0 ? 0 : 1; P.dst = last ? -1 : 1; P.flags = MRF_RES | MRF_KEEP;
        if (n > 2) return;
      }
// ... 86 lines not shown
```

piper_amd/csrc/kernels/col4.h:

```cpp
#pragma once
#include "dds.h"

namespace pe {

__device__ __forceinline__ int c4_tile(int bx, int nx, int P) { return pe_xcd_tile(bx, nx, P); }

constexpr int FFN_MAXS = 16;
constexpr int C4_H = 192, C4_NT = C4_H / 64;
template <int K>
struct Col4W {
  static constexpr int NQ = K / 16;
  static constexpr int KS = K + 4;
  f32x4 w[C4_NT][K / 16];
};
template <int K>
__device__ __forceinline__ void col_gemm4_fetch(Col4W<K>& W, const float* wp4, int nt, int wv, int lane) {
  constexpr int NQ = Col4W<K>::NQ, tile_floats = (K / 4) * 256;
#pragma unroll
  for (int m = 0; m < C4_NT; ++m) {
    const bool live = PE_UNIFORM(m < nt);
    const pe_rowsrc ws = pe_make_row_u(wp4 + (long)(live ? m : 0) * tile_floats, live ? tile_floats : 0);
#pragma unroll
    for (int q = 0; q < NQ; ++q) W.w[m][q] = pe_row_load4(ws, ((NQ * wv + q) * 64 + lane) * 4);
  }
  PE_SCHED_FENCE();
}
template <int K>
__device__ __forceinline__ void col_gemm4_run(const Col4W<K>& W, const float* YT, float* P, int wv, int lane) {
  constexpr int NQ = Col4W<K>::NQ, KS = Col4W<K>::KS;
  f32x4 acc[C4_NT];
#pragma unroll
  for (int m = 0; m < C4_NT; ++m)
#pragma unroll
    for (int r = 0; r < 4; ++r) acc[m][r] = 0.f;
  const float* yp = YT + (lane & 3) * KS + 4 * NQ * wv;
#pragma unroll
  for (int q = 0; q < NQ; ++q) {
    f32x4 yv;
#pragma unroll
    for (int j = 0; j < 4; ++j) yv[j] = yp[4 * q + j];
#pragma unroll
    for (int j = 0; j < 4; ++j)
#pragma unroll
      for (int m = 0; m < C4_NT; ++m) acc[m] = pe_mfma_4x4x1(W.w[m][q][j], yv[j], acc[m]);
  }
#pragma unroll
  for (int m = 0; m < C4_NT; ++m)
#pragma unroll
    for (int r = 0; r < 4; ++r) P[((wv * C4_NT + m) * 64 + 4 * (lane >> 2) + r) * 4 + (lane & 3)] = acc[m][r];
}
__device__ __forceinline__ float col_gemm4_get(const float* P, int c, int col) {
  const int o = c * 4 + col;
  return ((P[o] + P[C4_H * 4 + o]) + P[2 * C4_H * 4 + o]) + P[3 * C4_H * 4 + o];
}
__device__ __forceinline__ float pe_col_sum4(float v, float* red, int& flip, int wv, int lane, int col) {
  v += __shfl_xor(v, 4);
  v += __shfl_xor(v, 8);
  v += __shfl_xor(v, 16);
  v += __shfl_xor(v, 32);
  float* r = red + flip * 16;
  flip ^= 1;
  if (lane < 4) r[wv * 4 + col] = v;
  __syncthreads();
  return ((r[col] + r[4 + col]) + r[8 + col]) + r[12 + col];
}


template <bool FRONT>
__global__ __launch_bounds__(256) void colchain4_kernel(const int* lens, const float* in1, long in1_bs, int nx, int xcd, int mode,
                                                        int in1_cs, int K1r, int rows1, int first, int out_cs, ColP p) {
  PE_KTRACE(3);
  constexpr int NC = 4, NVT = 3, K1 = C4_H, K2 = C4_H / 2, KS1 = Col4W<K1>::KS, KS2 = Col4W<K2>::KS;
  PE_DYN_SMEM(float, sm);
  if constexpr (!FRONT) PE_STAMP(3, 0);
  p.lens = lens; p.xcd = xcd; p.mode = mode; p.in1 = in1; p.in1_bs = in1_bs; p.in1_cs = in1_cs; p.K1 = K1r; p.rows1 = rows1;
  p.first = first; p.out_cs = out_cs;
  const int b = blockIdx.y;
  int L = PE_UNIFORM(lens[b]);
  if constexpr (FRONT) PE_ENTRY_BATCH(L, p.res, p.res_bs, p.res_cs, p.gamma, p.beta, p.out, p.out_bs, p.x1, p.x1_bs, p.x1_cs, p.b1, p.w1,
                                      p.in0, p.in0_bs, p.in0_cs, p.w0, p.b0);
  else PE_ENTRY_BATCH(L, p.res, p.res_bs, p.res_cs, p.gamma, p.beta, p.out, p.out_bs, p.x1, p.x1_bs, p.x1_cs, p.b1, p.w1);
  const int t0 = c4_tile(blockIdx.x, nx, p.xcd) * NC;
  if (t0 >= L) return;
  if constexpr (!FRONT) PE_STAMP(3, 1);
  float* YT = sm;
  float* P = YT + NC * KS1;
  float* red = P + 4 * C4_H * NC;
  const int tid = threadIdx.x, col = tid & 3, rl = tid >> 2, wv = PE_UNIFORM(tid >> 6), lane = tid & 63;
  const int t = t0 + col;
  const bool ok = t < L;
  const int part = p.mode >= 2 ? (int)blockIdx.z : 0, row0 = part * C4_H;
  const int rows_here = p.rows1 - row0 < C4_H ? p.rows1 - row0 : C4_H;
  Col4W<K1> gw0;
  Col4W<K1> gw;
  auto fetch_gw = [&]() { col_gemm4_fetch<K1>(gw, p.w1 + (long)part * C4_NT * (K1 / 4) * 256, (rows_here + 63) / 64, wv, lane); };
  const bool skip_part = p.mode == 2 && (p.rows1 <= C4_H || part == 1);
  float sk[NVT];
  if constexpr (FRONT) {
    const pe_rowsrc a0 = pe_make_row(p.in0 + (long)b * p.in0_bs, K1 * p.in0_cs);
    const pe_rowsrc s0 = pe_make_row(p.in1 + (long)b * p.in1_bs, p.first ? 0 : K1 * p.in1_cs);
    const pe_rowsrc b0d = pe_make_row(p.b0 ? p.b0 : p.w0, p.b0 ? K1 : 0);
    float av[NVT], b0v[NVT];
#pragma unroll
    for (int k = 0; k < NVT; ++k) {
      const int c = rl + 64 * k;
      av[k] = pe_row_load(a0, ok ? c * p.in0_cs + t : -1);
      sk[k] = pe_row_load(s0, ok ? c * p.in1_cs + t : -1);
      b0v[k] = pe_row_load(b0d, c);
    }
    PE_SCHED_FENCE();
    col_gemm4_fetch<K1>(gw0, p.w0, C4_NT, wv, lane);
#pragma unroll
    for (int k = 0; k < NVT; ++k) YT[col * KS1 + rl + 64 * k] = av[k];
    __syncthreads();
    fetch_gw();
    col_gemm4_run<K1>(gw0, YT, P, wv, lane);
    __syncthreads();
#pragma unroll
    for (int k = 0; k < NVT; ++k) sk[k] = ok ? (col_gemm4_get(P, rl + 64 * k, col) + b0v[k]) + sk[k] : 0.f;
  }

  float ov[NVT], gg[NVT], bb[NVT], b1v[NVT];
  {
    const pe_rowsrc ind = pe_make_row(p.in1 + (long)b * p.in1_bs, p.K1 * p.in1_cs);
    const float* obp = p.mode == 0 ? p.res + (long)b * p.res_bs : (skip_part ? p.out + (long)b * p.out_bs : p.x1 + (long)b * p.x1_bs);
    const int ocs = p.mode == 0 ? p.res_cs : (skip_part ? p.out_cs : p.x1_cs);
    const pe_rowsrc od = p.mode == 3 ? pe_make_row(p.res ? p.res + (long)b * p.res_bs + row0 : p.w1, p.res ? rows_here : 0)
                                     : pe_make_row(obp, (skip_part && p.first) ? 0 : rows_here * ocs);
    const pe_rowsrc gd = pe_make_row(p.mode == 0 ? p.gamma : p.w1, p.mode == 0 ? p.rows1 : 0);
    const pe_rowsrc bd = pe_make_row(p.mode == 0 ? p.beta : p.w1, p.mode == 0 ? p.rows1 : 0);
    const pe_rowsrc b1d = pe_make_row(p.b1 ? p.b1 + row0 : p.w1, p.b1 ? rows_here : 0);
    float xin[NVT];
#pragma unroll
    for (int k = 0; k < NVT; ++k) {
      const int c = rl + 64 * k;
      xin[k] = FRONT ? sk[k] : pe_row_load(ind, ok ? c * p.in1_cs + t : -1);
      ov[k] = pe_row_load(od, (ok && c < rows_here) ? (p.mode == 3 ? c : c * ocs + t) : -1);
      gg[k] = pe_row_load(gd, c < rows_here ? c : -1);
      bb[k] = pe_row_load(bd, c < rows_here ? c : -1);
      b1v[k] = pe_row_load(b1d, c < rows_here ? c : -1);
    }
    PE_SCHED_FENCE();
    if constexpr (!FRONT) fetch_gw();
    if constexpr (!FRONT) PE_STAMP(3, 2);
#pragma unroll
    for (int k = 0; k < NVT; ++k) YT[col * KS1 + rl + 64 * k] = xin[k];
  }
  __syncthreads();
  col_gemm4_run<K1>(gw, YT, P, wv, lane);
  Col4W<K2> gw2;
  const bool second = p.mode == 1 && p.w2;
  if (second) col_gemm4_fetch<K2>(gw2, p.w2, (p.rows2 + 63) / 64, wv, lane);
  __syncthreads();

  if (p.mode >= 2) {
    if (!ok) return;
    float* tp = (skip_part || p.mode == 3) ? p.out + (long)b * p.out_bs + (p.mode == 3 ? (long)row0 * p.out_cs : 0) : p.x1 + (long)b * p.x1_bs;
    const int tcs = (skip_part || p.mode == 3) ? p.out_cs : p.x1_cs;
#pragma unroll
    for (int k = 0; k < NVT; ++k) {
      const int c = rl + 64 * k;
      if (c < rows_here) {
        const float val = (col_gemm4_get(P, c, col) + b1v[k]) + ov[k];
        tp[(long)c * tcs + t] = val;
        if (p.mode == 3 && p.kT && part == 1) p.kT[(long)b * p.kt_bs + ((long)(c >> 2) * p.out_cs + t) * 4 + (c & 3)] = val;
        if (p.mode == 3 && p.vQ && part == 2) p.vQ[(long)b * p.kt_bs + ((long)(t >> 2) * C4_H + c) * 4 + (t & 3)] = val;
      }
    }
    return;
  }
  if (p.mode == 0) {
    int red_flip = 0;
    auto col_sum = [&](float x) -> float { return pe_col_sum4(x, red, red_flip, wv, lane, col); };
    const int H = p.rows1;
    float v[NVT];
    float s = 0.f;
#pragma unroll
    for (int k = 0; k < NVT; ++k) {
      const int c = rl + 64 * k;
      v[k] = (ok && c < H) ? (col_gemm4_get(P, c, col) + b1v[k]) + ov[k] : 0.f;
      s += v[k];
    }
    const float mean = col_sum(s) / (float)H;
    float q = 0.f;
#pragma unroll
    for (int k = 0; k < NVT; ++k)
      if (rl + 64 * k < H) { const float d = v[k] - mean; q = fmaf(d, d, q); }
    const float rstd = 1.f / sqrtf(col_sum(q) / (float)H + 1e-5f);
    if (!ok) return;
    float* ob = p.out + (long)b * p.out_bs;
#pragma unroll
    for (int k = 0; k < NVT; ++k) {
      const int c = rl + 64 * k;
      if (c < H) ob[(long)c * p.out_cs + t] = (v[k] - mean) * rstd * gg[k] + bb[k];
    }
    return;
  }

  {
    float* xb = p.x1 + (long)b * p.x1_bs;
    float* YT2 = YT;
    const pe_rowsrc b2d = pe_make_row(second ? p.b2 : p.w1, (second && p.b2) ? p.rows2 : 0);
    float b2v[NVT];
#pragma unroll
    for (int k = 0; k < NVT; ++k) b2v[k] = pe_row_load(b2d, rl + 64 * k);
#pragma unroll
    for (int k = 0; k < NVT; ++k) {
      const int c = rl + 64 * k;
      if (c < K2) {
        const float xn = (ok && c < p.rows1) ? ov[k] - (col_gemm4_get(P, c, col) + b1v[k]) : 0.f;
        if (ok && c < p.rows1) xb[(long)c * p.x1_cs + t] = xn;
        YT2[col * KS2 + c] = xn;
      }
    }
    if (!second) return;
    __syncthreads();
    col_gemm4_run<K2>(gw2, YT2, P, wv, lane);
    __syncthreads();
    if (!ok) return;
    float* o2 = p.out2 + (long)b * p.o2_bs;
#pragma unroll
    for (int k = 0; k < NVT; ++k) {
      const int c = rl + 64 * k;
      if (c < p.rows2) o2[(long)c * p.o2_cs + t] = col_gemm4_get(P, c, col) + b2v[k];
    }
  }
}

__global__ __launch_bounds__(256) void lngemm4_kernel(const int* lens, int nx, int xcd, const float* in, long in_bs, int in_cs,
                                                      int rows, const float* parts, int nparts, LnGemmP p) {
  PE_KTRACE(7);
  constexpr int NC = 4, NVT = 3, H = C4_H, KS = Col4W<H>::KS;
  PE_DYN_SMEM(float, sm);
  p.lens = lens; p.xcd = xcd; p.in = in; p.in_bs = in_bs; p.in_cs = in_cs; p.rows = rows; p.parts = parts; p.nparts = nparts;
  const int b = blockIdx.y;
  int L = PE_UNIFORM(lens[b]);
  PE_ENTRY_BATCH(L, p.gamma, p.beta, p.bias, p.pbias, p.p_bs, p.w16);
  const int t0 = c4_tile(blockIdx.x, nx, p.xcd) * NC;
  if (t0 >= L) return;
  float* YT = sm;
  float* P = YT + NC * KS;
  float* red = P + 4 * H * NC;
  const int tid = threadIdx.x, col = tid & 3, rl = tid >> 2, wv = PE_UNIFORM(tid >> 6), lane = tid & 63;
  const int t = t0 + col;
  const bool ok = t < L;
  const int part = blockIdx.z, row0 = part * H;
  const int rows_here = p.rows - row0 < H ? p.rows - row0 : H;
  Col4W<H> gw;
  auto fetch_gw = [&]() { col_gemm4_fetch<H>(gw, p.w16 + (long)part * C4_NT * (H / 4) * 256, (rows_here + 63) / 64, wv, lane); };
  float v[NVT], gg[NVT], bb[NVT], cb[NVT];
  {
    const pe_rowsrc ind = pe_make_row(p.in + (long)b * p.in_bs, H * p.in_cs);
    const pe_rowsrc gd = pe_make_row(p.gamma, H), bd = pe_make_row(p.beta, H);
    const pe_rowsrc cbd = pe_make_row(p.bias ? p.bias + row0 : p.gamma, p.bias ? rows_here : 0);
#pragma unroll
    for (int k = 0; k < NVT; ++k) {
      const int c = rl + 64 * k;
      v[k] = pe_row_load(ind, ok ? c * p.in_cs + t : -1);
      gg[k] = pe_row_load(gd, c);
      bb[k] = pe_row_load(bd, c);
      cb[k] = pe_row_load(cbd, c);
    }
    if (p.parts) {
      const pe_rowsrc pbd = pe_make_row(p.pbias, H);
      float pv[NVT][FFN_MAXS];
      float pbv[NVT];
#pragma unroll
      for (int k = 0; k < NVT; ++k) {
        const int c = rl + 64 * k;
        pbv[k] = pe_row_load(pbd, c);
        const pe_rowsrc pd = pe_make_row(p.parts + (long)b * p.p_bs + (long)(t0 >> 2) * p.nparts * (H * 4), p.nparts * (H * 4));
#pragma unroll
        for (int sl = 0; sl < FFN_MAXS; ++sl) pv[k][sl] = pe_row_load(pd, (ok && sl < p.nparts) ? sl * (H * 4) + c * 4 + col : -1);
      }
      PE_SCHED_FENCE();
      fetch_gw();
#pragma unroll
      for (int k = 0; k < NVT; ++k) {
        float a = pv[k][0];
#pragma unroll
        for (int sl = 1; sl < FFN_MAXS; ++sl) a += pv[k][sl];
        v[k] = ok ? v[k] + (a + pbv[k]) : 0.f;
      }
    } else {
      PE_SCHED_FENCE();
      fetch_gw();
    }
  }
  int red_flip = 0;
  auto col_sum = [&](float x) -> float { return pe_col_sum4(x, red, red_flip, wv, lane, col); };
  float s = 0.f;
#pragma unroll
  for (int k = 0; k < NVT; ++k) s += v[k];
  const float mean = col_sum(s) / (float)H;
  float q = 0.f;
#pragma unroll
  for (int k = 0; k < NVT; ++k) { const float d = v[k] - mean; q = fmaf(d, d, q); }
  const float rstd = 1.f / sqrtf(col_sum(q) / (float)H + 1e-5f);
  float* xo = p.xout + (long)b * p.x_bs;
#pragma unroll
  for (int k = 0; k < NVT; ++k) {
    const int c = rl + 64 * k;
    const float y = ok ? (v[k] - mean) * rstd * gg[k] + bb[k] : 0.f;
// ... 25 lines not shown
```

piper_amd/csrc/kernels/gate4.h:

```cpp
#pragma once
#include "conv_common.h"

namespace pe {

constexpr int G4_NC = 12, G4_WC = 16, G4_NW = 12, G4_K = 192, G4_XS = G4_K + 4;
__global__ __launch_bounds__(64 * G4_NW) void gate4_kernel(const int* lens, int len_mul, const float* x, long x_bs, int x_cs,
                                                           int Cin, int padl, int ntaps_, const float* wpg4, ConvP p) {
  PE_KTRACE(4);
  PE_DYN_SMEM(float, sm);
  p.lens = lens; p.len_mul = len_mul; p.x = x; p.x_bs = x_bs; p.x_cs = x_cs; p.Cin = Cin; p.padl = padl; p.ntaps = ntaps_;
  p.wpg4 = wpg4;
  float* XT = sm;
  float* P = XT + G4_WC * G4_XS;
  const int b = blockIdx.z, grp = blockIdx.y;
  PE_STAMP(5, 0);
  const int L = p.lens[b] * p.len_mul;
  const int n0 = blockIdx.x * G4_NC;
  const int tid = threadIdx.x, lane = tid & 63, wv = PE_UNIFORM(tid >> 6);
  const int l3 = lane & 3, lb = lane >> 2;
  const int ntaps = p.ntaps;
  const pe_rowsrc xd = pe_make_row(p.x + (long)b * p.x_bs, p.Cin * p.x_cs);
  float xv[4];
#pragma unroll
  for (int u = 0; u < 4; ++u) {
    const int idx = tid + 64 * G4_NW * u, ch = idx >> 4, c = idx & 15, t = n0 - p.padl + c;
    xv[u] = pe_row_load(xd, (t >= 0 && t < p.x_cs) ? ch * p.x_cs + t : -1);
  }
  PE_SCHED_FENCE();
  f32x4 wf[5][4];
  {
    const int tap_floats = (G4_K / 4) * 256;
    const pe_rowsrc wd = pe_make_row_u(p.wpg4 + (long)grp * ntaps * tap_floats, ntaps * tap_floats);
#pragma unroll
    for (int tp = 0; tp < 5; ++tp)
#pragma unroll
      for (int q = 0; q < 4; ++q) wf[tp][q] = pe_row_load4(wd, tp < ntaps ? ((tp * (G4_K / 4) + 4 * wv + q) * 64 + lane) * 4 : -4);
  }
  PE_SCHED_FENCE();
  if (n0 >= L) return;
  PE_STAMP(5, 1);
  {
    const float slope = p.in_slope;
#pragma unroll
    for (int u = 0; u < 4; ++u) {
      const int idx = tid + 64 * G4_NW * u, ch = idx >> 4, c = idx & 15, t = n0 - p.padl + c;
      float v = (t < L) ? xv[u] : 0.f;
      if (slope != 1.f) v = pe_lrelu(v, slope);
      XT[c * G4_XS + ch] = v;
    }
  }
  __syncthreads();
  PE_STAMP(5, 2);
  {
    f32x4 acc[3];
#pragma unroll
    for (int g = 0; g < 3; ++g)
#pragma unroll
      for (int r = 0; r < 4; ++r) acc[g][r] = 0.f;
    const float* xp = XT + l3 * G4_XS + 16 * wv;
#pragma unroll
    for (int tp = 0; tp < 5; ++tp) {
      if (tp < ntaps) {
#pragma unroll
        for (int q = 0; q < 4; ++q) {
          f32x4 b4[3];
#pragma unroll
          for (int g = 0; g < 3; ++g) b4[g] = *reinterpret_cast<const f32x4*>(xp + (4 * g + tp) * G4_XS + 4 * q);
#pragma unroll
          for (int j = 0; j < 4; ++j)
#pragma unroll
            for (int g = 0; g < 3; ++g) acc[g] = pe_mfma_4x4x1(wf[tp][q][j], b4[g][j], acc[g]);
        }
      }
    }
#pragma unroll
    for (int g = 0; g < 3; ++g)
#pragma unroll
      for (int r = 0; r < 4; ++r) P[(wv * 64 + 4 * lb + r) * G4_NC + 4 * g + l3] = acc[g][r];
  }
  PE_STAMP(5, 3);
  __syncthreads();
  PE_STAMP(5, 4);
  if (tid < 32 * G4_NC) {
    const int c = tid / G4_NC, col = tid - c * G4_NC;
    const int ch = grp * 32 + c, t = n0 + col;
    if (ch < p.split && t < L) {
      float ta = 0.f, sa = 0.f;
#pragma unroll
      for (int w = 0; w < G4_NW; ++w) {
        ta += P[(w * 64 + c) * G4_NC + col];
        sa += P[(w * 64 + 32 + c) * G4_NC + col];
      }
      conv_store_gate(p, b, ch, t, ta, sa);
    }
  }
  PE_STAMP(5, 5);
}

}
```

piper_amd/csrc/kernels/launch.h:

```cpp
#pragma once
#include "../pe_rt.h"
#include "params.h"

namespace pe {
namespace launch {

void init_conv();
void conv_tile(int cfg, bool gate, int halo, dim3 grid, size_t smem, hipStream_t stream, const ConvP& p);
void conv1x1(dim3 grid, hipStream_t stream, const ConvP& p);
void conv_splitk(bool gate, int nw, dim3 grid, size_t smem, hipStream_t stream, const ConvP& p);
void conv_splitk16(bool gate, dim3 grid, size_t smem, hipStream_t stream, const ConvP& p, bool half = false);
void gate4(dim3 grid, size_t smem, hipStream_t stream, const ConvP& p);
void conv_group(bool wide, dim3 grid, size_t smem, hipStream_t stream, const ConvG& g);
void conv_tile_group(int cfg, int halo, dim3 grid, size_t smem, hipStream_t stream, const ConvG& g);
void conv_group_sum(dim3 grid, size_t smem, hipStream_t stream, const ConvP& p);

void init_bf3();
void conv_bf3(int sm, int cfg, bool gate, int halo, dim3 grid, size_t smem, hipStream_t stream, const ConvP& p);
void mrf_split(int sm, int cp, int ou, dim3 grid, hipStream_t stream, const MrfP& p);

void init_front();
void embed(dim3 grid, hipStream_t stream, const EmbedP& p);
void attention(int dk, dim3 grid, size_t smem, hipStream_t stream, const AttnP& p);
void attno(dim3 grid, size_t smem, hipStream_t stream, const AttnOP& p);
void attn4(bool long_rows, dim3 grid, size_t smem, hipStream_t stream, const AttnOP& p);
void layer_norm(dim3 grid, hipStream_t stream, const LnP& p);
void dds_layer(int nchunks, dim3 grid, size_t smem, hipStream_t stream, const DdsP& p);
void dds_layer4(dim3 grid, size_t smem, hipStream_t stream, const DdsP& p);
void colchain(dim3 grid, size_t smem, hipStream_t stream, const ColP& p);
void colchain4(dim3 grid, size_t smem, hipStream_t stream, const ColP& p);
void lngemm(dim3 grid, size_t smem, hipStream_t stream, const LnGemmP& p);
void lngemm4(dim3 grid, size_t smem, hipStream_t stream, const LnGemmP& p);
void ffn(dim3 grid, size_t smem, hipStream_t stream, const FfnP& p);
void cf_pre(dim3 grid, hipStream_t stream, const float* z0, long z_bs, const float* w, const float* bias, const float* xg,
            long g_bs, int g_cs, float* out, long o_bs, int o_cs, const int* lens, int H);
void spline_inverse(dim3 grid, hipStream_t stream, const float* hproj, long h_bs, int h_cs, float* z1, long z_bs,
                    const int* lens, float inv_sqrt_h);
void scale(dim3 grid, hipStream_t stream, const float* in, float* out, long n, const float* s, long per_utt);
void duration(dim3 grid, hipStream_t stream, const DurP& p);
void duration_plan(dim3 grid, hipStream_t stream, const PlanP& p);
void randn(hipStream_t stream, float* out, long rows, int cols, long stride, long row0, const unsigned long long* state,
           int site, const unsigned long long* keys = nullptr, const int* use = nullptr, int ch = 1);
void regulate(dim3 grid, hipStream_t stream, const RegP& p);
void xcc_probe(hipStream_t stream, int* out64);
void cond(dim3 grid, hipStream_t stream, const float* emb_g, int gin, const int* sids, const float* w, const float* bias,
          int rows, float* out, int o_bs);
void speaker_blend(hipStream_t stream, int batch, const BlendP& p);

void init_tail();
void mrf(int cp, int ou, dim3 grid, hipStream_t stream, const MrfP& p);
void mrf_sum(dim3 grid, hipStream_t stream, const float* r0, const float* r1, const float* r2, float* out, long bs, int cs,
             const int* lens, int len_mul, float scale);
void conv_post(dim3 grid, hipStream_t stream, const float* x, long x_bs, int x_cs, const float* w, int Cin, float slope,
               const int* lens, int len_mul, float* audio, long a_bs, unsigned* absmax);
void pcm16(dim3 grid, hipStream_t stream, const float* audio, long a_bs, const unsigned* absmax, const int* lens,
           int len_mul, short* pcm, long p_bs, short* host);
void window_copy(dim3 grid, hipStream_t stream, const float* z, int zs, const int* win, float* out, int ws, int C);
void window_gather(dim3 grid, hipStream_t stream, const float* z, long z_bs, int zs, const int* hst, int* dst, int cap,
                   float* out, long o_bs, int ws, int wg);
void chunk_peak(dim3 grid, hipStream_t stream, const float* audio, long a_bs, int* st, int cap, int hop);
void chunk_pcm(dim3 grid, hipStream_t stream, const float* audio, long a_bs, const int* st, int cap, int hop);
void stream_gain(hipStream_t stream, int* ctl, int* gb, int cap, int B, int mode, const int* st, int hop, const int* rows,
                 int rcap, long y_cap);
void chunk_pcm_gain(dim3 grid, hipStream_t stream, const float* audio, long a_bs, const int* st, int cap, int hop, const int* gq);
void stream_adopt(dim3 grid, hipStream_t stream, const float* z, long z_bs, int zs, const float* cond, int cond_bs,
                  int cond_rows, const int* join, int cap, float* pool, long p_bs, int ps, float* pcond, int slots);
void resample_rows(hipStream_t stream, const int* hst, const int* lens, int len_mul, int* rows, int cap, int B, long x_cap,
                   long y_cap, int L, int M);
void resample(dim3 grid, hipStream_t stream, const RsP& p);
void chunk_pcm_rs(dim3 grid, hipStream_t stream, const float* y, long y_bs, const int* rows, int rcap, const int* st, int cap);
void chunk_pcm_rs_gain(dim3 grid, hipStream_t stream, const float* y, long y_bs, const int* rows, int rcap, const int* st, int cap,
                       const int* gq);
void loudness_seg(dim3 grid, hipStream_t stream, const LoudP& p);
void true_peak(dim3 grid, hipStream_t stream, const TpP& p);
void loudness_gain(hipStream_t stream, int B, const double* seg, int nseg_cap, const int* lens, int len_mul, long x_cap, int h,
                   const unsigned* peaks, const unsigned* tpeaks, int* ctl, int* gd, int cap, int limiter);
void limiter(dim3 grid, hipStream_t stream, const LimP& p);
void true_peak_v(dim3 grid, hipStream_t stream, const TpP& p);
void limiter_true(dim3 grid, hipStream_t stream, const LimP& p);
void pcm16_trim(dim3 grid, hipStream_t stream, const TrimP& p);
void pcm16_gain(dim3 grid, hipStream_t stream, const float* audio, long a_bs, const int* gq, int gcap, const int* lens,
                int len_mul, short* pcm, long p_bs, short* host);

}
}
```

piper_amd/csrc/kernels/launch_conv.cpp:

```cpp
#include "launch.h"

#include "conv_mfma.h"
#include "conv1x1.h"
#include "conv_splitk.h"
#include "gate4.h"

namespace pe {
namespace launch {

void init_conv() {
#ifndef PE_EMU
  const int lim = 160 * 1024;
#define PE_K2(WM, WN, MT, NT, KS, G) (const void*)conv_mfma_kernel<WM, WN, MT, NT, KS, G, 64>, (const void*)conv_mfma_kernel<WM, WN, MT, NT, KS, G, 128>
  const void* ks[] = {PE_K2(1, 4, 1, 1, 16, false), PE_K2(2, 2, 1, 1, 16, false), PE_K2(1, 4, 2, 1, 16, true),
                      PE_K2(2, 2, 2, 1, 16, true),
                      (const void*)conv_mfma_group_kernel<2, 2, 1, 1, 16, 64>, (const void*)conv_mfma_group_kernel<2, 2, 1, 1, 16, 128>,
                      (const void*)conv_mfma_group_kernel<1, 4, 1, 1, 16, 64>, (const void*)conv_mfma_group_kernel<1, 4, 1, 1, 16, 128>,
                      (const void*)conv_splitk_kernel<2, true, 8, 3>, (const void*)conv_splitk_kernel<2, true, 4, 3>,
                      (const void*)conv_splitk_kernel<1, false, 8, 4>, (const void*)conv_splitk_kernel<1, false, 4, 4>,
                      (const void*)conv_splitk_kernel<2, true, 12, 2>, (const void*)conv_splitk_kernel<1, false, 12, 4>,
                      (const void*)conv_splitk16_kernel<true, 12, 2>, (const void*)conv_splitk16_kernel<false, 8, 4>,
                      (const void*)conv_splitk_group_kernel<4, 2, 64>, (const void*)conv_splitk_group_kernel<4, 2, 128>,
                      (const void*)conv_splitk_sum_kernel<4, 2>};
#undef PE_K2
  for (const void* k : ks) PE_HIP(hipFuncSetAttribute(k, hipFuncAttributeMaxDynamicSharedMemorySize, lim));
#endif
}

void conv_tile(int cfg, bool gate, int halo, dim3 grid, size_t smem, hipStream_t stream, const ConvP& p) {
#define PE_CT_ARGS p.lens, p.x, p.x_bs, p.len_mul, p.epi, p.tpb, p.x_cs, p.Cin, p.padl, p.ntaps, p.nchunks, p
#define PE_CONV_LAUNCH(WM, WN, MT, NT, KS, G)                                                                  \
  do {                                                                                                         \
    if (halo == 64) PE_LAUNCH((conv_mfma_kernel<WM, WN, MT, NT, KS, G, 64>), grid, dim3(256), smem, stream, PE_CT_ARGS); \
    else PE_LAUNCH((conv_mfma_kernel<WM, WN, MT, NT, KS, G, 128>), grid, dim3(256), smem, stream, PE_CT_ARGS);          \
  } while (0)
  if (gate) {
    if (cfg == 1) PE_CONV_LAUNCH(1, 4, 2, 1, 16, true);
    else PE_CONV_LAUNCH(2, 2, 2, 1, 16, true);
  } else {
    if (cfg == 2) PE_CONV_LAUNCH(1, 4, 1, 1, 16, false);
    else PE_CONV_LAUNCH(2, 2, 1, 1, 16, false);
  }
#undef PE_CONV_LAUNCH
#undef PE_CT_ARGS
}

void conv_tile_group(int cfg, int halo, dim3 grid, size_t smem, hipStream_t stream, const ConvG& g) {
  if (cfg == 2) {
    if (halo == 64) PE_LAUNCH((conv_mfma_group_kernel<1, 4, 1, 1, 16, 64>), grid, dim3(256), smem, stream, g);
    else PE_LAUNCH((conv_mfma_group_kernel<1, 4, 1, 1, 16, 128>), grid, dim3(256), smem, stream, g);
  } else {
    if (halo == 64) PE_LAUNCH((conv_mfma_group_kernel<2, 2, 1, 1, 16, 64>), grid, dim3(256), smem, stream, g);
    else PE_LAUNCH((conv_mfma_group_kernel<2, 2, 1, 1, 16, 128>), grid, dim3(256), smem, stream, g);
  }
}

void conv1x1(dim3 grid, hipStream_t stream, const ConvP& p) { PE_LAUNCH((conv1x1_kernel<1>), grid, dim3(256), 0, stream, p); }

void conv_splitk(bool gate, int nw, dim3 grid, size_t smem, hipStream_t stream, const ConvP& p) {
#define PE_SK_ARGS p.lens, p.x, p.x_bs, p.x_cs, p.Cin, p.padl, p.ntaps, p.nchunks, p.tgroups, p.wp, p
  if (gate) {
    if (nw == 12) PE_LAUNCH((conv_splitk_kernel<2, true, 12, 2>), grid, dim3(768), smem, stream, PE_SK_ARGS);
    else if (nw == 8) PE_LAUNCH((conv_splitk_kernel<2, true, 8, 3>), grid, dim3(512), smem, stream, PE_SK_ARGS);
    else PE_LAUNCH((conv_splitk_kernel<2, true, 4, 3>), grid, dim3(256), smem, stream, PE_SK_ARGS);
  } else {
    if (nw == 12) PE_LAUNCH((conv_splitk_kernel<1, false, 12, 4>), grid, dim3(768), smem, stream, PE_SK_ARGS);
    else if (nw == 8) PE_LAUNCH((conv_splitk_kernel<1, false, 8, 4>), grid, dim3(512), smem, stream, PE_SK_ARGS);
    else PE_LAUNCH((conv_splitk_kernel<1, false, 4, 4>), grid, dim3(256), smem, stream, PE_SK_ARGS);
  }
#undef PE_SK_ARGS
}

void conv_splitk16(bool gate, dim3 grid, size_t smem, hipStream_t stream, const ConvP& p, bool half) {
#define PE_SK_ARGS p.lens, p.x, p.x_bs, p.x_cs, p.Cin, p.padl, p.ntaps, p.nchunks, p.tgroups, p.wp16, p
  if (gate && half) PE_LAUNCH((conv_splitk16_kernel<true, 6, 5, 2>), grid, dim3(64 * 6), smem, stream, PE_SK_ARGS);
  else if (gate) PE_LAUNCH((conv_splitk16_kernel<true, 12, 2>), grid, dim3(64 * 12), smem, stream, PE_SK_ARGS);
  else PE_LAUNCH((conv_splitk16_kernel<false, 8, 4>), grid, dim3(64 * 8), smem, stream, PE_SK_ARGS);
#undef PE_SK_ARGS
}

void gate4(dim3 grid, size_t smem, hipStream_t stream, const ConvP& p) {
  PE_LAUNCH(gate4_kernel, grid, dim3(64 * G4_NW), smem, stream, p.lens, p.len_mul, p.x, p.x_bs, p.x_cs, p.Cin, p.padl, p.ntaps, p.wpg4, p);
}

void conv_group(bool wide, dim3 grid, size_t smem, hipStream_t stream, const ConvG& g) {
  if (wide) PE_LAUNCH((conv_splitk_group_kernel<4, 2, 128>), grid, dim3(256), smem, stream, g.B, g);
  else PE_LAUNCH((conv_splitk_group_kernel<4, 2, 64>), grid, dim3(256), smem, stream, g.B, g);
}

void conv_group_sum(dim3 grid, size_t smem, hipStream_t stream, const ConvP& p) {
  PE_LAUNCH((conv_splitk_sum_kernel<4, 2>), grid, dim3(256), smem, stream, p);
}

}
}

#ifdef PE_STAMPS
PE_TRACE_FETCHER(conv)
#endif
```

piper_amd/csrc/policy.cpp:

```cpp
#include "policy.h"

#include <cerrno>
#include <cstdio>
#include <cstdlib>
#include <cstring>
#include <mutex>
#include <stdexcept>
#include <string>

namespace pe {

static const LaunchPolicy::Knob kKnobs[] = {
    {"PIPER_HIP_MRF", &LaunchPolicy::mrf, 0, 2, "fused MRF stage kernel: 0 off (conv by conv), 1 by the measured policy (ResBlock2 stages always; ResBlock1 stages on 32 channels up to PIPER_HIP_MRF_MAXF frames per call), 2 wherever it applies"},
    {"PIPER_HIP_MRF_MAXF", &LaunchPolicy::mrf_maxf, 0, 1L << 40, "batch frames up to which a 32-channel ResBlock1 stage runs in the fused kernel (mode 1)"},
    {"PIPER_HIP_MRF_OU", &LaunchPolicy::mrf_ou, 0, 4, "force the output units per wave of mrf_kernel (1..4) instead of the cost model; ignored when the width does not fit"},
    {"PIPER_HIP_MRF_TAIL", &LaunchPolicy::mrf_tail, 0, 1, "generator tail inside the last stage's mrf_kernel (0: separate conv_post_kernel)"},
    {"PIPER_HIP_MRF_SPLIT", &LaunchPolicy::mrf_split, 0, 1, "matrix modes bf16x3 / f16x3: the fused MRF stage kernel on the 16-bit matrix pipe with split operands (mrf_split_kernel) wherever a fused stage applies; 0 = the f32 fused kernel below PIPER_HIP_BF3_MINF frames, conv by conv on the 16-bit pipe above"},
    {"PIPER_HIP_BF3_MINF", &LaunchPolicy::bf3_minf, 0, 1L << 40, "split matrix modes without a fused 16-bit stage kernel (bf16x6, or PIPER_HIP_MRF_SPLIT=0): batch frames from which the <= 64-channel MRF stages run conv by conv on the 16-bit pipe"},
    {"PIPER_HIP_SPLITK_MAX", &LaunchPolicy::splitk_max, 0, 1L << 40, "tile-workgroup count below which a conv goes to the split-K kernels (0: always the tiled kernel)"},
    {"PIPER_HIP_SPLITK16", &LaunchPolicy::splitk16, 0, 3, "16-column split-K form: 0 off, 1 gate convs, 2 + long-K plain convs, 3 everywhere"},
    {"PIPER_HIP_WIDE_SPLITK", &LaunchPolicy::wide_splitk, 0, 2, "12-wave split-K: 0 off, 1 WN gate conv, 2 always"},
    {"PIPER_HIP_TPB", &LaunchPolicy::tpb, 0, 64, "tiled kernel: column tiles walked by one workgroup (0 = 1)"},
    {"PIPER_HIP_GROUP_MRF", &LaunchPolicy::group_mrf, 0, 2, "sibling resblock convs of a wider small stage as grouped launches (one-utterance calls): 0 off, 2 without the K-concatenated last step"},
    {"PIPER_HIP_GROUP_MAXB", &LaunchPolicy::group_maxb, 0, 1L << 40, "64 x 64 tiles of one conv of a stage below which the grouped sibling launches of a single utterance take the split-K kernels (the tiled grouped launches from there on)"},
    {"PIPER_HIP_GROUP_TILED", &LaunchPolicy::group_tiled, 0, 1, "sibling resblock convs of a stage that runs the tiled kernel as grouped launches (conv_mfma_group_kernel) while one conv is at most 2048 tile workgroups (8 per CU): 0 = one launch per conv"},
    {"PIPER_HIP_COLCHAIN", &LaunchPolicy::colchain, 0, 2, "colchain_kernel / lngemm_kernel: 0 off, 1 up to 4096 ids / 8192 frames per call, 2 always"},
    {"PIPER_HIP_COL4", &LaunchPolicy::col4, 0, 2, "4-column forms of the 192-channel chains: 0 off, 1 up to PIPER_HIP_COL4_MAXC ids (2048 frames for the flow's launches) per call, 2 always"},
    {"PIPER_HIP_COL4_MAXC", &LaunchPolicy::col4_maxc, 0, 1L << 40, "ids per call up to which the 4-column chains are used"},
    {"PIPER_HIP_FFN", &LaunchPolicy::ffn, 0, 1, "the encoder FFN as one launch (ffn_kernel) wherever the 4-column chains run: 0 = conv by conv"},
    {"PIPER_HIP_ATTNO", &LaunchPolicy::attno, 0, 1, "attention + conv_o + norm_layers_1 as one launch (attno_kernel) wherever the 4-column chains run: 0 = attn_kernel + colchain4_kernel"},
    {"PIPER_HIP_ATTN4", &LaunchPolicy::attn4, 0, 2, "attention + conv_o + norm_layers_1 on 4-query workgroups (attn4_kernel) in place of attno_kernel: 0 off, 1 for calls whose longest utterance has up to PIPER_HIP_ATTN4_MAXC ids, 2 wherever attno_kernel applies"},
    {"PIPER_HIP_ATTN4_MAXC", &LaunchPolicy::attn4_maxc, 0, 1L << 40, "ids of the longest utterance of a call up to which attention runs on 4-query workgroups"},
    {"PIPER_HIP_FUSE_DP", &LaunchPolicy::fuse_dp, 0, 1, "ConvFlow.pre / proj / spline fused into the DDSConv layer launches"},
    {"PIPER_HIP_SPEC", &LaunchPolicy::spec, 0, 1, "speculative stage-B sizing / whole utterance as one graph for <= 4 utterances per call"},
    {"PIPER_HIP_SPEC_EXPECT", &LaunchPolicy::spec_expect, 0, 1, "speculative graphs planned for the expected frame counts (0: for the bucket capacity)"},
    {"PIPER_HIP_PCM_ZC", &LaunchPolicy::pcm_zc, 0, 1, "PCM written straight into pinned host memory by pcm16_kernel (0: one copy per utterance behind the graph)"},
    {"PIPER_HIP_IDS_ZC", &LaunchPolicy::ids_zc, 0, 1, "phoneme ids, lengths and speaker ids read straight from the pinned host block by embed_kernel, up to 65536 padded ids per call (0: one host-to-device copy in front of the graph)"},
    {"PIPER_HIP_NO_GRAPH", &LaunchPolicy::no_graph, 0, 1, "launch kernels directly instead of replaying hipGraphs"},
    {"PIPER_HIP_GRAPHS", &LaunchPolicy::graphs, 1, 4096, "hipGraphs kept per engine (least recently used evicted one at a time)"},
    {"PIPER_HIP_CONVT_VEC", &LaunchPolicy::convt_vec, 0, 1, "polyphase up-conv: a lane's four accumulator rows leave as one 16-byte store (stride a multiple of 4) or two 8-byte stores (stride 2) of consecutive output samples; 0: one 4-byte store per phase"},
    {"PIPER_HIP_XCD", &LaunchPolicy::xcd, -1, 32, "XCDs the dispatch round-robins over, for the XCD-aware tile orders (-1 = probed at engine creation, 0 = tiles in workgroup order)"},
    {"PIPER_HIP_XCD_FFN", &LaunchPolicy::xcd_ffn, 0, 1, "ffn_kernel deals (column tile, slice) to the XCDs slice-major, so an XCD's L2 holds two slices' weights instead of all sixteen (0: blockIdx order)"},
    {"PIPER_HIP_STACK_PRE", &LaunchPolicy::stack_pre, 0, 1, "small calls of the 192-channel voices: enc_p.proj and dp.pre (both read the last LayerNorm's output) as one lngemm4_kernel launch over the stacked matrix (0: two launches)"},
    {"PIPER_HIP_CHAIN_RS", &LaunchPolicy::chain_rs, 0, 1, "small calls of the 192-channel voices: the last WN layer's res/skip conv (skip rows only) in front of the coupling layer's post + pre chain launch, colchain4_kernel<true> (0: a launch of its own)"},
    {"PIPER_HIP_GATE4", &LaunchPolicy::gate4, 0, 2, "short calls: the WN gate conv over 192 channels on 64-row x 12-column workgroups with the 4x4x1 MFMA (gate4_kernel) up to 640 workgroups: 0 off (16-column split-K form), 2 wherever the split-K route applies"},
    {"PIPER_HIP_GATE_HALF", &LaunchPolicy::gate_half, 0, 1, "short one-utterance calls (up to 128 whole-group workgroups): the WN gate conv on half a 32-channel group per workgroup, six waves with the whole K range in flight, twice the workgroups (0: whole groups on twelve waves)"},
    {"PIPER_HIP_CONV1X1", &LaunchPolicy::conv1x1, 0, 1, "batched one-tap convs (q/k/v, WN res/skip, coupling pre/post, proj) through conv1x1_kernel, B operand straight from global memory (0: the tiled kernel)"},
    {"PIPER_HIP_WS_BUDGET_MB", &LaunchPolicy::ws_budget_mb, 0, 1048576, "MiB of device memory the workspace of one pipeline half may take (0: a third of the device's memory): capacities grow only inside it, a call that does not fit by itself is an error"},
    {"PIPER_HIP_ATTN_LONG", &LaunchPolicy::attn_long, 0, 1, "attention score slabs in global memory (attn_long_kernel) at every length, also in place of attno_kernel (tests): by default only utterances whose 32 x T slab does not fit LDS (more than ~830 ids) take that form"},
    {"PIPER_HIP_PROF_SITES", &LaunchPolicy::prof_sites, 0, 1, "level-2 profile rows of the tiled conv kernel per conv shape (tuning aid)"},
    {"PIPER_HIP_DEBUG_KEEP", &LaunchPolicy::debug_keep, 0, 1, "test hook: keep z_p for pe_debug_tensor"},
    {"PIPER_HIP_DEBUG_POISON", &LaunchPolicy::debug_poison, 0, 1, "test hook: activation workspaces are filled with NaN bit patterns when allocated (no kernel may read what the call did not write)"},
};

const LaunchPolicy::Knob* LaunchPolicy::knobs(int* n) {
  if (n) *n = (int)(sizeof(kKnobs) / sizeof(kKnobs[0]));
  return kKnobs;
}

void LaunchPolicy::read_env() {
  for (const Knob& k : kKnobs) {
    const char* t = getenv(k.env);
    if (!t || !*t) continue;
    errno = 0;
    char* end = nullptr;
    const long v = strtol(t, &end, 10);
    if (errno || end == t || *end)
      throw std::runtime_error(std::string(k.env) + "=" + t + ": not an integer (" + k.doc + ")");
    this->*k.field = v < k.lo ? k.lo : (v > k.hi ? k.hi : v);
  }
}

int LaunchPolicy::matrix_mode_env() {
  const char* t = getenv("PIPER_HIP_MATRIX");
  if (!t || !t[0] || !strcmp(t, "f32")) return -1;
  if (!strcmp(t, "bf16x3")) return 0;
  if (!strcmp(t, "f16x3")) return 1;
  if (!strcmp(t, "bf16x6")) return 2;
  throw std::runtime_error("PIPER_HIP_MATRIX: expected f32, bf16x3, f16x3 or bf16x6");
}

const char* LaunchPolicy::describe() {
  static std::string out;
  static std::once_flag once;
  std::call_once(once, [] {
    const LaunchPolicy d;
    out = "[";
    for (const Knob& k : kKnobs) {
      char head[160];
      snprintf(head, sizeof(head), "%s{\"env\":\"%s\",\"default\":%ld,\"lo\":%ld,\"hi\":%ld,\"doc\":\"", out.size() > 1 ? "," : "", k.env,
               d.*k.field, k.lo, k.hi);
      out += head;
      for (const char* c = k.doc; *c; ++c) {
        if (*c == '"' || *c == '\\') out += '\\';
        out += *c;
      }
      out += "\"}";
    }
    out += "]";
  });
  return out.c_str();
}

}
```

piper_amd/csrc/policy.h:

```cpp
#pragma once
#include <cstddef>

namespace pe {

struct LaunchPolicy {
  long mrf = 1;
  long mrf_maxf = 1100;
  long mrf_ou = 0;
  long mrf_tail = 1;
  long mrf_split = 1;
  long bf3_minf = 1100;
  long splitk_max = 96;
  long splitk16 = 2;
  long wide_splitk = 1;
  long tpb = 0;
  long group_mrf = 1;
  long group_maxb = 160;
  long group_tiled = 1;
  long colchain = 1;
  long col4 = 1;
  long col4_maxc = 1024;
  long ffn = 1;
  long attno = 1;
  long attn4 = 1;
  long attn4_maxc = 512;
  long fuse_dp = 1;
  long spec = 1;
  long spec_expect = 1;
  long pcm_zc = 1;
  long ids_zc = 1;
  long no_graph = 0;
  long graphs = 256;
  long convt_vec = 1;
  long xcd = -1;
  long xcd_ffn = 1;
  long stack_pre = 1;
  long chain_rs = 1;
  long gate4 = 1;
  long gate_half = 1;
  long conv1x1 = 1;
  long ws_budget_mb = 0;
  long attn_long = 0;
  long prof_sites = 0;
  long debug_keep = 0;
  long debug_poison = 0;

  static constexpr long colchain_max_ids = 4096, colchain_max_frames = 8192;
  static constexpr long col4_max_frames = 2048;
  static constexpr long ffn_max_cols = 2048;
  static constexpr int spec_max_batch = 4;
  static constexpr long ids_zc_max = 65536;
  static constexpr long group_max_blocks64 = 700;
  static constexpr long group_tiled_max_blocks = 2048;

  struct Knob { const char* env; long LaunchPolicy::*field; long lo, hi; const char* doc; };
  static const Knob* knobs(int* n);
  void read_env();
  static const char* describe();
  static int matrix_mode_env();
  static bool matrix_bf3_env() { return matrix_mode_env() >= 0; }

  bool splitk(long blocks, int halo, int cin) const { return blocks < splitk_max && halo <= 32 && cin % 32 == 0; }
  bool groupable(bool gate, bool convt, long blocks, int halo, int cin) const {
    return !gate && !convt && blocks < splitk_max && halo <= 96 && cin % 32 == 0;
  }
  bool splitk_16col(bool packed16, bool convt, bool gate, int units) const {
    return packed16 && !convt && ((gate && splitk16 >= 1) || (!gate && splitk16 >= 2)) && (units >= 24 || splitk16 >= 3);
  }
  bool splitk_12wave(bool gate, int units, int nchunks, int ntaps) const {
    return (wide_splitk == 1 && gate && units >= 24 && nchunks <= 6 && ntaps >= 4) || wide_splitk == 2;
  }
  bool one_tap_direct(bool gate, bool convt, int ntaps, int cin) const {
    return conv1x1 && !gate && !convt && ntaps == 1 && cin % 32 == 0;
  }
  bool gate_half_groups(bool gate, int nchunks, int ntaps, long workgroups_whole) const {
    return gate_half && gate && nchunks == 6 && ntaps <= 5 && 2 * workgroups_whole <= 256;
  }
  static constexpr long gate4_max_workgroups = 640;
  bool gate_12col(bool gate, bool packed4, int ntaps, int dil, long workgroups) const {
    return gate4 && gate && packed4 && ntaps <= 5 && dil == 1 && (gate4 == 2 || workgroups <= gate4_max_workgroups);
  }
  int tiles_per_workgroup() const { return tpb > 0 ? (int)tpb : 1; }
  bool chain16(double cols, bool frames, int k1, int half) const {
    return colchain && k1 == 192 && half == 96 && (colchain == 2 || cols <= (double)(frames ? colchain_max_frames : colchain_max_ids));
  }
  bool chain4(long cols, long limit = 0) const { return col4 && (col4 == 2 || cols <= (limit ? limit : col4_maxc)); }
  bool attn4_ids(long longest_utterance) const { return attn4 == 2 || (attn4 == 1 && longest_utterance <= attn4_maxc); }
  bool chain4_frames(long cols) const { return chain4(cols, col4_max_frames); }
  bool chain_rs_front(long cols) const { return chain_rs && chain4_frames(cols); }
  bool mrf_build(int channels) const { return mrf != 0 && channels <= 64 && channels % 4 == 0; }
  bool mrf_stage(bool built, bool resblock1, int padded_channels, double frames, bool matrix_bf3, bool split_fused = false) const {
    if (mrf && built && split_fused) return mrf == 2 || !resblock1 || padded_channels == 32;
    return mrf && built && !(matrix_bf3 && mrf != 2 && frames >= (double)bf3_minf) &&
           (mrf == 2 || !resblock1 || (padded_channels == 32 && frames <= (double)mrf_maxf));
  }
  bool group_stage(int B, int nk, long blocks64, bool buffers_fit) const {
    return group_mrf && B == 1 && nk >= 2 && nk <= 3 && blocks64 < group_max_blocks64 && blocks64 < group_maxb && buffers_fit;
  }
  bool stage_all_tiled(int B, int nk, long blocks64) const {
    return group_mrf && group_tiled && B == 1 && nk >= 2 && nk <= 3 && blocks64 >= group_maxb;
  }
  bool group_sum() const { return group_mrf != 2; }
  bool group_stage_tiled(int nk, long tile_blocks, bool buffers_fit) const {
    return group_tiled && nk >= 2 && nk <= 3 && tile_blocks <= group_tiled_max_blocks && buffers_fit;
  }
  bool speculate(int B) const { return spec && !no_graph && B <= spec_max_batch; }
  bool ids_from_host(long padded_ids) const { return ids_zc && padded_ids <= ids_zc_max; }
};

}
```

Before: 123.3 million samples/s.

## Compose coupling-layer pre 1x1 conv into first WN gate conv weights

Precomputes on the host the product of each coupling layer's pre 1x1 weight with the first WN gate conv weight, plus per-tap bias terms for the edges, and runs a new gate4pre kernel straight on the 96-channel half input. The separate pre conv launch and the chain's pre GEMM are dropped. The first res/skip colchain launch also computes the pre term of the hidden state through a second accumulated GEMM. This cuts launches and K work in the flow but adds edge-bias handling and extra host-side packing, with rounding that differs from the unfused path.

```diff
diff --git a/piper_amd/csrc/engine.h b/piper_amd/csrc/engine.h
--- a/piper_amd/csrc/engine.h
+++ b/piper_amd/csrc/engine.h
@@ -260,6 +260,9 @@
                     double flops, const float* bias2 = nullptr, long bias2_bs = 0, const float* w4direct = nullptr, int kin = 192,
                     long max_cols = 0);
   const float* pack4_conv_pad192(const WeightSet& ws, const std::string& wname, int in_rev, int out_rev);
+  struct Rcl;
+  void pack_gate4pre(const WeightSet& ws, const std::string& prefix, bool odd, Rcl& r);
+  void gate_pre(const Rcl& r, View x0, View out, const int* lens, int Lmax, double cols, const float* b2);
   struct LnSecond { const float* w4 = nullptr; int split = 0; View out2{nullptr, 0, 0}; const float* bias2 = nullptr; long bias2_bs = 0; };
   void lngemm(View y, const float* g, const float* b, View x, const float* w16, const float* bias, int rows, View out,
               int T, double flops, const float* parts = nullptr, int nparts = 0, const float* pbias = nullptr,
@@ -331,6 +334,7 @@
     const float* pre4pad = nullptr;
     std::vector<PackedConv> in, rs;
     std::vector<const float*> rs4;
+    const float* gpre4 = nullptr; const float* gpre_bias = nullptr; const float* gpre_tapb = nullptr;
     int in_off, out_off;
   };
   std::vector<Rcl> rcls_;
diff --git a/piper_amd/csrc/engine_issue.cpp b/piper_amd/csrc/engine_issue.cpp
--- a/piper_amd/csrc/engine_issue.cpp
+++ b/piper_amd/csrc/engine_issue.cpp
@@ -310,22 +310,35 @@
   const View fh = VF(fh_, H_), facts = VF(facts_, H_), fskip = VF(fskip_, H_);
   const int half = C_ / 2;
   const bool chain = pol_.chain16(fsum, true, H_, half);
+  auto rs_front_of = [&](size_t ri, bool front = true) {
+    const Rcl& r = rcls_[ri];
+    const int nl = (int)r.in.size();
+    return chain && nl >= 1 && r.rs4[nl - 1] && r.rs[nl - 1].rows == H_ && H_ == 192 && half == 96 &&
+           (front ? pol_.chain_rs_front((long)B * Fmax) : pol_.chain4_frames((long)B * Fmax)) && w4_of(r.post16) &&
+           (ri + 1 >= rcls_.size() || (rcls_[ri + 1].pre.rows <= 192 && w4_of(rcls_[ri + 1].pre16)));
+  };
+  auto compose_pre_of = [&](size_t ri) {
+    if (ri >= rcls_.size() || !pol_.compose_pre() || !rs_front_of(ri, false)) return false;
+    const Rcl& r = rcls_[ri];
+    return r.in.size() >= 2 && r.gpre4 && r.rs4[0] && r.rs[0].rows == 2 * H_ && w4_of(r.pre16) && r.pre.rows == H_ &&
+           plan_conv(r.in[0], Fmax, EPI_GATE, stage_tiled_).form == CONV_GATE12;
+  };
   for (size_t ri = 0; ri < rcls_.size(); ++ri) {
     Rcl& r = rcls_[ri];
     const View x0{zp_ + (long)r.in_off * Fs, (long)C_ * Fs, Fs};
     const View x1{zp_ + (long)r.out_off * Fs, (long)C_ * Fs, Fs};
-    if (!(chain && ri > 0)) {
+    const bool compose_pre = compose_pre_of(ri);
+    if (!(chain && ri > 0) && !compose_pre) {
       if (!(chain && r.pre4pad && conv1x1_col4(nullptr, r.pre.bias, r.pre.rows, x0, fh, lens_b_, B, Fmax, 2.0 * fsum * r.pre.macs_per_col,
                                                nullptr, 0, r.pre4pad, half, LaunchPolicy::col4_max_frames)))
         conv(r.pre, x0, fh, lens_b_, 1, Fmax, EPI_STORE);
     }
     const int nl = (int)r.in.size();
-    const bool rs_front = chain && nl >= 1 && r.rs4[nl - 1] && r.rs[nl - 1].rows == H_ && H_ == 192 && half == 96 &&
-                          pol_.chain_rs_front((long)B * Fmax) && w4_of(r.post16) &&
-                          (ri + 1 >= rcls_.size() || (rcls_[ri + 1].pre.rows <= 192 && w4_of(rcls_[ri + 1].pre16)));
+    const bool rs_front = rs_front_of(ri);
     for (int i = 0; i < nl; ++i) {
       const float* b2 = nspk_ > 1 ? cond_ + cond_off_wn_[ri] + (long)i * 2 * H_ : nullptr;
-      conv(r.in[i], fh, facts, lens_b_, 1, Fmax, EPI_GATE, {.bias2 = b2, .bias2_bs = cond_bs_});
+      if (compose_pre && i == 0) gate_pre(r, x0, facts, lens_b_, Fmax, fsum, b2);
+      else conv(r.in[i], fh, facts, lens_b_, 1, Fmax, EPI_GATE, {.bias2 = b2, .bias2_bs = cond_bs_});
       if (rs_front && i == nl - 1) {
         fl += 2.0 * fsum * (r.in[i].macs_per_col + r.rs[i].macs_per_col);
         continue;
@@ -339,9 +352,15 @@
         cp.x1 = fh.p; cp.x1_bs = fh.bs; cp.x1_cs = fh.cs;
         cp.out = fskip.p; cp.out_bs = fskip.bs; cp.out_cs = fskip.cs;
         cp.lens = lens_b_;
-        const int kh4 = kbegin(prof_level_ >= 2 ? krow("colchain4_kernel<false>") : 0, 2.0 * fsum * r.rs[i].macs_per_col,
-                               4.0 * (fsum * (H_ + 2.0 * cp.rows1) + (double)cp.rows1 * H_));
-        launch::colchain4(dim3((Fmax + 3) / 4, B, (cp.rows1 + 191) / 192), col4_smem(), stream_, cp);
+        const bool hpre = compose_pre && i == 0;
+        if (hpre) {
+          cp.in0 = x0.p; cp.in0_bs = x0.bs; cp.in0_cs = x0.cs;
+          cp.w2 = w4_of(r.pre16); cp.b2 = r.pre.bias; cp.rows2 = H_;
+        }
+        const int kh4 = kbegin(prof_level_ >= 2 ? krow("colchain4_kernel<false>") : 0,
+                               2.0 * fsum * (r.rs[i].macs_per_col + (hpre ? r.pre.macs_per_col : 0)),
+                               4.0 * (fsum * (H_ + 2.0 * cp.rows1) + (double)cp.rows1 * H_ + (hpre ? half * (fsum + H_) : 0)));
+        launch::colchain4(dim3((Fmax + 3) / 4, B, (cp.rows1 + 191) / 192), col4_smem() + (hpre ? 4 * (96 + 4) * sizeof(float) : 0), stream_, cp);
         kend(kh4);
       } else {
         conv(r.rs[i], facts, fh, lens_b_, 1, Fmax, EPI_WNRS, {.out2 = fskip, .mode = i == 0 ? 1 : 0});
@@ -354,7 +373,7 @@
       cp.w1 = r.post16; cp.b1 = r.post.bias; cp.rows1 = half;
       cp.mode = 1;
       cp.x1 = x1.p; cp.x1_bs = x1.bs; cp.x1_cs = x1.cs;
-      if (ri + 1 < rcls_.size()) {
+      if (ri + 1 < rcls_.size() && !compose_pre_of(ri + 1)) {
         const Rcl& nx = rcls_[ri + 1];
         if (nx.in_off != r.out_off) throw std::runtime_error("coupling layers do not alternate halves");
         cp.w2 = nx.pre16; cp.b2 = nx.pre.bias; cp.rows2 = H_;
diff --git a/piper_amd/csrc/engine_launch.cpp b/piper_amd/csrc/engine_launch.cpp
--- a/piper_amd/csrc/engine_launch.cpp
+++ b/piper_amd/csrc/engine_launch.cpp
@@ -268,6 +268,22 @@
     case CONV_1X1: launch::conv1x1(pl.grid, ls_, p); break;
     case CONV_TILE: launch::conv_tile(pl.cfg, pc.gate, pl.halo, pl.grid, pl.smem, ls_, p); break;
   }
+  kend(kh);
+}
+
+void Engine::gate_pre(const Rcl& r, View x0, View out, const int* lens, int Lmax, double cols, const float* b2) {
+  const PackedConv& pc = r.in[0];
+  ConvP p{};
+  p.x = x0.p; p.x_bs = x0.bs; p.x_cs = x0.cs;
+  p.wpg4 = r.gpre4; p.bias = r.gpre_bias;
+  p.bias2 = b2; p.bias2_bs = cond_bs_;
+  p.out = out.p; p.o_bs = out.bs; p.o_cs = out.cs;
+  p.lens = lens; p.len_mul = 1;
+  p.Cin = 96; p.rows = pc.rows; p.ntaps = pc.ntaps; p.dil = 1; p.padl = pc.padl; p.xhalo = pc.ntaps - 1;
+  p.in_slope = 1.f; p.epi = EPI_GATE; p.split = pc.split;
+  const double macs = (double)pc.rows * 96 * pc.ntaps;
+  const int kh = kbegin(prof_level_ >= 2 ? krow("gate4pre_kernel") : 0, 2.0 * macs * cols, 4.0 * (cols * (96 + pc.split) + macs));
+  launch::gate4pre(dim3((Lmax + 11) / 12, pc.split / 32, B_), ((size_t)16 * (96 + 4) + (size_t)6 * 64 * 12) * sizeof(float), ls_, p, r.gpre_tapb);
   kend(kh);
 }
 
diff --git a/piper_amd/csrc/engine_pack.cpp b/piper_amd/csrc/engine_pack.cpp
--- a/piper_amd/csrc/engine_pack.cpp
+++ b/piper_amd/csrc/engine_pack.cpp
@@ -335,6 +335,48 @@
   return pack4(W, Co, 192);
 }
 
+void Engine::pack_gate4pre(const WeightSet& ws, const std::string& prefix, bool odd, Rcl& r) {
+  const HostTensor& wg = ws.get(prefix + ".enc.in_layers.0.weight");
+  const HostTensor& wp = ws.get(prefix + ".pre.weight");
+  if (wg.dims.size() != 3 || wp.dims.size() != 3 || wp.dims[2] != 1) return;
+  const int R = (int)wg.dims[0], H = (int)wg.dims[1], nt = (int)wg.dims[2], Ci = (int)wp.dims[1], split = R / 2;
+  if (H != 192 || (int)wp.dims[0] != H || Ci != 96 || nt > 5 || R != 2 * H || !r.in[0].wpg4) return;
+  const std::string bgn = prefix + ".enc.in_layers.0.bias", bpn = prefix + ".pre.bias";
+  const size_t n4 = (size_t)(split / 32) * nt * (Ci / 4) * 256;
+  std::vector<float> G(skeleton_ ? 0 : n4, 0.f), bsum(skeleton_ ? 0 : R, 0.f), tapb(skeleton_ ? 0 : (size_t)6 * R, 0.f);
+  if (!skeleton_) {
+    std::vector<double> P((size_t)H * Ci), bp(H, 0.0), acc(Ci);
+    for (int c = 0; c < H; ++c)
+      for (int i = 0; i < Ci; ++i) P[(size_t)c * Ci + i] = wp.data[(size_t)c * Ci + (odd ? Ci - 1 - i : i)];
+    if (ws.has(bpn))
+      for (int c = 0; c < H; ++c) bp[c] = ws.get(bpn).data[c];
+    const bool has_bg = ws.has(bgn);
+    for (int row = 0; row < R; ++row) {
+      const int ch = row < split ? row : row - split, g = ch / 32, lane = (ch & 31) + (row < split ? 0 : 32);
+      double bs = has_bg ? (double)ws.get(bgn).data[row] : 0.0;
+      tapb[(size_t)5 * R + row] = (float)bs;
+      for (int k = 0; k < nt; ++k) {
+        std::fill(acc.begin(), acc.end(), 0.0);
+        double bk = 0.0;
+        for (int c = 0; c < H; ++c) {
+          const double a = wg.data[((size_t)row * H + c) * nt + k];
+          const double* pr = &P[(size_t)c * Ci];
+          for (int i = 0; i < Ci; ++i) acc[i] += a * pr[i];
+          bk += a * bp[c];
+        }
+        for (int i = 0; i < Ci; ++i)
+          G[((((size_t)g * nt + k) * (Ci / 4) + i / 4) * 64 + lane) * 4 + (i & 3)] = (float)acc[i];
+        tapb[(size_t)k * R + row] = (float)bk;
+        bs += bk;
+      }
+      bsum[row] = (float)bs;
+    }
+  }
+  r.gpre4 = dev_alloc(n4, skeleton_ ? nullptr : G.data());
+  r.gpre_bias = dev_alloc((size_t)R, skeleton_ ? nullptr : bsum.data());
+  r.gpre_tapb = dev_alloc((size_t)6 * R, skeleton_ ? nullptr : tapb.data());
+}
+
 DdsW Engine::load_dds(const WeightSet& ws, const std::string& p) {
   DdsW d;
   for (int i = 0; i < arch_[A_DDSLAYERS]; ++i) {
@@ -486,6 +528,7 @@
       r.pre16 = pack16_conv(ws, p + ".pre.weight", odd, 0);
       if (H_ == 192 && rcls_.empty()) r.pre4pad = pack4_conv_pad192(ws, p + ".pre.weight", odd, 0);
       r.post16 = pack16_conv(ws, p + ".post.weight", 0, odd);
+      if (wnl >= 2) pack_gate4pre(ws, p, odd, r);
       rcls_.push_back(r);
       if (gin_) {
         const HostTensor& cw = ws.get(p + ".enc.cond_layer.weight");
diff --git a/piper_amd/csrc/kernels/col4.h b/piper_amd/csrc/kernels/col4.h
--- a/piper_amd/csrc/kernels/col4.h
+++ b/piper_amd/csrc/kernels/col4.h
@@ -26,13 +26,8 @@
   PE_SCHED_FENCE();
 }
 template <int K>
-__device__ __forceinline__ void col_gemm4_run(const Col4W<K>& W, const float* YT, float* P, int wv, int lane) {
+__device__ __forceinline__ void col_gemm4_acc(const Col4W<K>& W, const float* YT, f32x4 (&acc)[C4_NT], int wv, int lane) {
   constexpr int NQ = Col4W<K>::NQ, KS = Col4W<K>::KS;
-  f32x4 acc[C4_NT];
-#pragma unroll
-  for (int m = 0; m < C4_NT; ++m)
-#pragma unroll
-    for (int r = 0; r < 4; ++r) acc[m][r] = 0.f;
   const float* yp = YT + (lane & 3) * KS + 4 * NQ * wv;
 #pragma unroll
   for (int q = 0; q < NQ; ++q) {
@@ -44,10 +39,34 @@
 #pragma unroll
       for (int m = 0; m < C4_NT; ++m) acc[m] = pe_mfma_4x4x1(W.w[m][q][j], yv[j], acc[m]);
   }
+}
+__device__ __forceinline__ void col_gemm4_zero(f32x4 (&acc)[C4_NT]) {
 #pragma unroll
   for (int m = 0; m < C4_NT; ++m)
 #pragma unroll
+    for (int r = 0; r < 4; ++r) acc[m][r] = 0.f;
+}
+__device__ __forceinline__ void col_gemm4_put(const f32x4 (&acc)[C4_NT], float* P, int wv, int lane) {
+#pragma unroll
+  for (int m = 0; m < C4_NT; ++m)
+#pragma unroll
     for (int r = 0; r < 4; ++r) P[((wv * C4_NT + m) * 64 + 4 * (lane >> 2) + r) * 4 + (lane & 3)] = acc[m][r];
+}
+template <int K>
+__device__ __forceinline__ void col_gemm4_run(const Col4W<K>& W, const float* YT, float* P, int wv, int lane) {
+  f32x4 acc[C4_NT];
+  col_gemm4_zero(acc);
+  col_gemm4_acc<K>(W, YT, acc, wv, lane);
+  col_gemm4_put(acc, P, wv, lane);
+}
+template <int K, int K2>
+__device__ __forceinline__ void col_gemm4_run2(const Col4W<K>& W, const float* YT, const Col4W<K2>& W2, const float* YT2, float* P,
+                                               int wv, int lane) {
+  f32x4 acc[C4_NT];
+  col_gemm4_zero(acc);
+  col_gemm4_acc<K>(W, YT, acc, wv, lane);
+  col_gemm4_acc<K2>(W2, YT2, acc, wv, lane);
+  col_gemm4_put(acc, P, wv, lane);
 }
 __device__ __forceinline__ float col_gemm4_get(const float* P, int c, int col) {
   const int o = c * 4 + col;
@@ -79,7 +98,8 @@
   int L = PE_UNIFORM(lens[b]);
   if constexpr (FRONT) PE_ENTRY_BATCH(L, p.res, p.res_bs, p.res_cs, p.gamma, p.beta, p.out, p.out_bs, p.x1, p.x1_bs, p.x1_cs, p.b1, p.w1,
                                       p.in0, p.in0_bs, p.in0_cs, p.w0, p.b0);
-  else PE_ENTRY_BATCH(L, p.res, p.res_bs, p.res_cs, p.gamma, p.beta, p.out, p.out_bs, p.x1, p.x1_bs, p.x1_cs, p.b1, p.w1);
+  else PE_ENTRY_BATCH(L, p.res, p.res_bs, p.res_cs, p.gamma, p.beta, p.out, p.out_bs, p.x1, p.x1_bs, p.x1_cs, p.b1, p.w1,
+                      p.in0, p.in0_bs, p.in0_cs, p.w2, p.b2, p.kT, p.kt_bs, p.vQ);
   const int t0 = c4_tile(blockIdx.x, nx, p.xcd) * NC;
   if (t0 >= L) return;
   if constexpr (!FRONT) PE_STAMP(3, 1);
@@ -95,6 +115,9 @@
   Col4W<K1> gw;
   auto fetch_gw = [&]() { col_gemm4_fetch<K1>(gw, p.w1 + (long)part * C4_NT * (K1 / 4) * 256, (rows_here + 63) / 64, wv, lane); };
   const bool skip_part = p.mode == 2 && (p.rows1 <= C4_H || part == 1);
+  const bool pre_part = !FRONT && p.mode == 2 && p.w2 && !skip_part;
+  float* YTP = P + 4 * C4_H * NC + 32 + 64 * 4;
+  Col4W<K2> gw2;
   float sk[NVT];
   if constexpr (FRONT) {
     const pe_rowsrc a0 = pe_make_row(p.in0 + (long)b * p.in0_bs, K1 * p.in0_cs);
@@ -126,7 +149,10 @@
     const float* obp = p.mode == 0 ? p.res + (long)b * p.res_bs : (skip_part ? p.out + (long)b * p.out_bs : p.x1 + (long)b * p.x1_bs);
     const int ocs = p.mode == 0 ? p.res_cs : (skip_part ? p.out_cs : p.x1_cs);
     const pe_rowsrc od = p.mode == 3 ? pe_make_row(p.res ? p.res + (long)b * p.res_bs + row0 : p.w1, p.res ? rows_here : 0)
+                         : pre_part  ? pe_make_row(p.b2 ? p.b2 : p.w1, p.b2 ? rows_here : 0)
                                      : pe_make_row(obp, (skip_part && p.first) ? 0 : rows_here * ocs);
+    const pe_rowsrc x0d = pe_make_row(p.in0 + (long)b * p.in0_bs, pre_part ? K2 * p.in0_cs : 0);
+    float x0v[2];
     const pe_rowsrc gd = pe_make_row(p.mode == 0 ? p.gamma : p.w1, p.mode == 0 ? p.rows1 : 0);
     const pe_rowsrc bd = pe_make_row(p.mode == 0 ? p.beta : p.w1, p.mode == 0 ? p.rows1 : 0);
     const pe_rowsrc b1d = pe_make_row(p.b1 ? p.b1 + row0 : p.w1, p.b1 ? rows_here : 0);
@@ -135,20 +161,27 @@
     for (int k = 0; k < NVT; ++k) {
       const int c = rl + 64 * k;
       xin[k] = FRONT ? sk[k] : pe_row_load(ind, ok ? c * p.in1_cs + t : -1);
-      ov[k] = pe_row_load(od, (ok && c < rows_here) ? (p.mode == 3 ? c : c * ocs + t) : -1);
+      ov[k] = pe_row_load(od, (ok && c < rows_here) ? ((p.mode == 3 || pre_part) ? c : c * ocs + t) : -1);
+      if (!FRONT && k < 2) x0v[k] = pe_row_load(x0d, (ok && c < K2) ? c * p.in0_cs + t : -1);
       gg[k] = pe_row_load(gd, c < rows_here ? c : -1);
       bb[k] = pe_row_load(bd, c < rows_here ? c : -1);
       b1v[k] = pe_row_load(b1d, c < rows_here ? c : -1);
     }
     PE_SCHED_FENCE();
     if constexpr (!FRONT) fetch_gw();
+    if (pre_part) col_gemm4_fetch<K2>(gw2, p.w2, C4_NT, wv, lane);
     if constexpr (!FRONT) PE_STAMP(3, 2);
 #pragma unroll
     for (int k = 0; k < NVT; ++k) YT[col * KS1 + rl + 64 * k] = xin[k];
-  }
-  __syncthreads();
-  col_gemm4_run<K1>(gw, YT, P, wv, lane);
-  Col4W<K2> gw2;
+    if constexpr (!FRONT)
+      if (pre_part) {
+        YTP[col * KS2 + rl] = x0v[0];
+        if (rl < K2 - 64) YTP[col * KS2 + rl + 64] = x0v[1];
+      }
+  }
+  __syncthreads();
+  if (pre_part) col_gemm4_run2<K1, K2>(gw, YT, gw2, YTP, P, wv, lane);
+  else col_gemm4_run<K1>(gw, YT, P, wv, lane);
   const bool second = p.mode == 1 && p.w2;
   if (second) col_gemm4_fetch<K2>(gw2, p.w2, (p.rows2 + 63) / 64, wv, lane);
   __syncthreads();
diff --git a/piper_amd/csrc/kernels/gate4.h b/piper_amd/csrc/kernels/gate4.h
--- a/piper_amd/csrc/kernels/gate4.h
+++ b/piper_amd/csrc/kernels/gate4.h
@@ -4,14 +4,13 @@
 namespace pe {
 
 constexpr int G4_NC = 12, G4_WC = 16, G4_NW = 12, G4_K = 192, G4_XS = G4_K + 4;
-__global__ __launch_bounds__(64 * G4_NW) void gate4_kernel(const int* lens, int len_mul, const float* x, long x_bs, int x_cs,
-                                                           int Cin, int padl, int ntaps_, const float* wpg4, ConvP p) {
-  PE_KTRACE(4);
+constexpr int G4P_K = 96, G4P_NW = G4P_K / 16;
+template <int K>
+__device__ __forceinline__ void gate4_body(ConvP& p, const float* tapb) {
+  constexpr int NW = K / 16, XS = K + 4;
   PE_DYN_SMEM(float, sm);
-  p.lens = lens; p.len_mul = len_mul; p.x = x; p.x_bs = x_bs; p.x_cs = x_cs; p.Cin = Cin; p.padl = padl; p.ntaps = ntaps_;
-  p.wpg4 = wpg4;
   float* XT = sm;
-  float* P = XT + G4_WC * G4_XS;
+  float* P = XT + G4_WC * XS;
   const int b = blockIdx.z, grp = blockIdx.y;
   PE_STAMP(5, 0);
   const int L = p.lens[b] * p.len_mul;
@@ -23,18 +22,18 @@
   float xv[4];
 #pragma unroll
   for (int u = 0; u < 4; ++u) {
-    const int idx = tid + 64 * G4_NW * u, ch = idx >> 4, c = idx & 15, t = n0 - p.padl + c;
+    const int idx = tid + 64 * NW * u, ch = idx >> 4, c = idx & 15, t = n0 - p.padl + c;
     xv[u] = pe_row_load(xd, (t >= 0 && t < p.x_cs) ? ch * p.x_cs + t : -1);
   }
   PE_SCHED_FENCE();
   f32x4 wf[5][4];
   {
-    const int tap_floats = (G4_K / 4) * 256;
+    const int tap_floats = (K / 4) * 256;
     const pe_rowsrc wd = pe_make_row_u(p.wpg4 + (long)grp * ntaps * tap_floats, ntaps * tap_floats);
 #pragma unroll
     for (int tp = 0; tp < 5; ++tp)
 #pragma unroll
-      for (int q = 0; q < 4; ++q) wf[tp][q] = pe_row_load4(wd, tp < ntaps ? ((tp * (G4_K / 4) + 4 * wv + q) * 64 + lane) * 4 : -4);
+      for (int q = 0; q < 4; ++q) wf[tp][q] = pe_row_load4(wd, tp < ntaps ? ((tp * (K / 4) + 4 * wv + q) * 64 + lane) * 4 : -4);
   }
   PE_SCHED_FENCE();
   if (n0 >= L) return;
@@ -43,10 +42,10 @@
     const float slope = p.in_slope;
 #pragma unroll
     for (int u = 0; u < 4; ++u) {
-      const int idx = tid + 64 * G4_NW * u, ch = idx >> 4, c = idx & 15, t = n0 - p.padl + c;
+      const int idx = tid + 64 * NW * u, ch = idx >> 4, c = idx & 15, t = n0 - p.padl + c;
       float v = (t < L) ? xv[u] : 0.f;
       if (slope != 1.f) v = pe_lrelu(v, slope);
-      XT[c * G4_XS + ch] = v;
+      XT[c * XS + ch] = v;
     }
   }
   __syncthreads();
@@ -57,7 +56,7 @@
     for (int g = 0; g < 3; ++g)
 #pragma unroll
       for (int r = 0; r < 4; ++r) acc[g][r] = 0.f;
-    const float* xp = XT + l3 * G4_XS + 16 * wv;
+    const float* xp = XT + l3 * XS + 16 * wv;
 #pragma unroll
     for (int tp = 0; tp < 5; ++tp) {
       if (tp < ntaps) {
@@ -65,7 +64,7 @@
         for (int q = 0; q < 4; ++q) {
           f32x4 b4[3];
 #pragma unroll
-          for (int g = 0; g < 3; ++g) b4[g] = *reinterpret_cast<const f32x4*>(xp + (4 * g + tp) * G4_XS + 4 * q);
+          for (int g = 0; g < 3; ++g) b4[g] = *reinterpret_cast<const f32x4*>(xp + (4 * g + tp) * XS + 4 * q);
 #pragma unroll
           for (int j = 0; j < 4; ++j)
 #pragma unroll
@@ -87,14 +86,50 @@
     if (ch < p.split && t < L) {
       float ta = 0.f, sa = 0.f;
 #pragma unroll
-      for (int w = 0; w < G4_NW; ++w) {
+      for (int w = 0; w < NW; ++w) {
         ta += P[(w * 64 + c) * G4_NC + col];
         sa += P[(w * 64 + 32 + c) * G4_NC + col];
       }
-      conv_store_gate(p, b, ch, t, ta, sa);
+      if constexpr (K == G4P_K) {
+        float bt = p.bias[ch], bs = p.bias[p.split + ch];
+        if (PE_UNIFORM(n0 < p.padl || n0 + G4_NC + ntaps - 1 - p.padl > L)) {
+          const int rs = 2 * p.split;
+          bt = tapb[5 * rs + ch];
+          bs = tapb[5 * rs + p.split + ch];
+          for (int k = 0; k < ntaps; ++k) {
+            const int u = t + k - p.padl;
+            if (u >= 0 && u < L) { bt += tapb[k * rs + ch]; bs += tapb[k * rs + p.split + ch]; }
+          }
+        }
+        ta += bt;
+        sa += bs;
+        if (p.bias2) {
+          const float* b2 = p.bias2 + (long)b * p.bias2_bs;
+          ta += b2[ch];
+          sa += b2[p.split + ch];
+        }
+        p.out[(long)b * p.o_bs + (long)ch * p.o_cs + t] = tanhf(ta) * (1.f / (1.f + expf(-sa)));
+      } else {
+        conv_store_gate(p, b, ch, t, ta, sa);
+      }
     }
   }
   PE_STAMP(5, 5);
 }
 
+__global__ __launch_bounds__(64 * G4_NW) void gate4_kernel(const int* lens, int len_mul, const float* x, long x_bs, int x_cs,
+                                                           int Cin, int padl, int ntaps_, const float* wpg4, ConvP p) {
+  PE_KTRACE(4);
+  p.lens = lens; p.len_mul = len_mul; p.x = x; p.x_bs = x_bs; p.x_cs = x_cs; p.Cin = Cin; p.padl = padl; p.ntaps = ntaps_;
+  p.wpg4 = wpg4;
+  gate4_body<G4_K>(p, nullptr);
 }
+__global__ __launch_bounds__(64 * G4P_NW) void gate4pre_kernel(const int* lens, int len_mul, const float* x, long x_bs, int x_cs,
+                                                               int padl, int ntaps_, const float* wpg4, const float* tapb, ConvP p) {
+  PE_KTRACE(4);
+  p.lens = lens; p.len_mul = len_mul; p.x = x; p.x_bs = x_bs; p.x_cs = x_cs; p.Cin = G4P_K; p.padl = padl; p.ntaps = ntaps_;
+  p.wpg4 = wpg4;
+  gate4_body<G4P_K>(p, tapb);
+}
+
+}
diff --git a/piper_amd/csrc/kernels/launch.h b/piper_amd/csrc/kernels/launch.h
--- a/piper_amd/csrc/kernels/launch.h
+++ b/piper_amd/csrc/kernels/launch.h
@@ -11,6 +11,7 @@
 void conv_splitk(bool gate, int nw, dim3 grid, size_t smem, hipStream_t stream, const ConvP& p);
 void conv_splitk16(bool gate, dim3 grid, size_t smem, hipStream_t stream, const ConvP& p, bool half = false);
 void gate4(dim3 grid, size_t smem, hipStream_t stream, const ConvP& p);
+void gate4pre(dim3 grid, size_t smem, hipStream_t stream, const ConvP& p, const float* tapb);
 void conv_group(bool wide, dim3 grid, size_t smem, hipStream_t stream, const ConvG& g);
 void conv_tile_group(int cfg, int halo, dim3 grid, size_t smem, hipStream_t stream, const ConvG& g);
 void conv_group_sum(dim3 grid, size_t smem, hipStream_t stream, const ConvP& p);
diff --git a/piper_amd/csrc/kernels/launch_conv.cpp b/piper_amd/csrc/kernels/launch_conv.cpp
--- a/piper_amd/csrc/kernels/launch_conv.cpp
+++ b/piper_amd/csrc/kernels/launch_conv.cpp
@@ -83,6 +83,10 @@
   PE_LAUNCH(gate4_kernel, grid, dim3(64 * G4_NW), smem, stream, p.lens, p.len_mul, p.x, p.x_bs, p.x_cs, p.Cin, p.padl, p.ntaps, p.wpg4, p);
 }
 
+void gate4pre(dim3 grid, size_t smem, hipStream_t stream, const ConvP& p, const float* tapb) {
+  PE_LAUNCH(gate4pre_kernel, grid, dim3(64 * G4P_NW), smem, stream, p.lens, p.len_mul, p.x, p.x_bs, p.x_cs, p.padl, p.ntaps, p.wpg4, tapb, p);
+}
+
 void conv_group(bool wide, dim3 grid, size_t smem, hipStream_t stream, const ConvG& g) {
   if (wide) PE_LAUNCH((conv_splitk_group_kernel<4, 2, 128>), grid, dim3(256), smem, stream, g.B, g);
   else PE_LAUNCH((conv_splitk_group_kernel<4, 2, 64>), grid, dim3(256), smem, stream, g.B, g);
diff --git a/piper_amd/csrc/policy.cpp b/piper_amd/csrc/policy.cpp
--- a/piper_amd/csrc/policy.cpp
+++ b/piper_amd/csrc/policy.cpp
@@ -44,6 +44,7 @@
     {"PIPER_HIP_STACK_PRE", &LaunchPolicy::stack_pre, 0, 1, "small calls of the 192-channel voices: enc_p.proj and dp.pre (both read the last LayerNorm's output) as one lngemm4_kernel launch over the stacked matrix (0: two launches)"},
     {"PIPER_HIP_CHAIN_RS", &LaunchPolicy::chain_rs, 0, 1, "small calls of the 192-channel voices: the last WN layer's res/skip conv (skip rows only) in front of the coupling layer's post + pre chain launch, colchain4_kernel<true> (0: a launch of its own)"},
     {"PIPER_HIP_GATE4", &LaunchPolicy::gate4, 0, 2, "short calls: the WN gate conv over 192 channels on 64-row x 12-column workgroups with the 4x4x1 MFMA (gate4_kernel) up to 640 workgroups: 0 off (16-column split-K form), 2 wherever the split-K route applies"},
+    {"PIPER_HIP_WN_COMPOSE", &LaunchPolicy::wn_compose, 0, 3, "short calls of the 192-channel voices, where the coupling chain runs on colchain4_kernel and the gate conv on gate4_kernel: 1x1 convs of a coupling layer composed into their neighbours when the weights are packed: 0 off, 1 every composition that is built, 2 only pre into the first gate conv (gate4pre_kernel over the 96 channels of x0; the coupling layer's pre launch and the chain's pre GEMM go, the first res/skip launch also writes the hidden state's pre term), 3 only post into the skip convs (not built: the route of 0)"},
     {"PIPER_HIP_GATE_HALF", &LaunchPolicy::gate_half, 0, 1, "short one-utterance calls (up to 128 whole-group workgroups): the WN gate conv on half a 32-channel group per workgroup, six waves with the whole K range in flight, twice the workgroups (0: whole groups on twelve waves)"},
     {"PIPER_HIP_CONV1X1", &LaunchPolicy::conv1x1, 0, 1, "batched one-tap convs (q/k/v, WN res/skip, coupling pre/post, proj) through conv1x1_kernel, B operand straight from global memory (0: the tiled kernel)"},
     {"PIPER_HIP_WS_BUDGET_MB", &LaunchPolicy::ws_budget_mb, 0, 1048576, "MiB of device memory the workspace of one pipeline half may take (0: a third of the device's memory): capacities grow only inside it, a call that does not fit by itself is an error"},
diff --git a/piper_amd/csrc/policy.h b/piper_amd/csrc/policy.h
--- a/piper_amd/csrc/policy.h
+++ b/piper_amd/csrc/policy.h
@@ -37,6 +37,7 @@
   long stack_pre = 1;
   long chain_rs = 1;
   long gate4 = 1;
+  long wn_compose = 1;
   long gate_half = 1;
   long conv1x1 = 1;
   long ws_budget_mb = 0;
@@ -88,6 +89,7 @@
   bool attn4_ids(long longest_utterance) const { return attn4 == 2 || (attn4 == 1 && longest_utterance <= attn4_maxc); }
   bool chain4_frames(long cols) const { return chain4(cols, col4_max_frames); }
   bool chain_rs_front(long cols) const { return chain_rs && chain4_frames(cols); }
+  bool compose_pre() const { return wn_compose == 1 || wn_compose == 2; }
   bool mrf_build(int channels) const { return mrf != 0 && channels <= 64 && channels % 4 == 0; }
   bool mrf_stage(bool built, bool resblock1, int padded_channels, double frames, bool matrix_bf3, bool split_fused = false) const {
     if (mrf && built && split_fused) return mrf == 2 || !resblock1 || padded_channels == 32;
```

New measurement: 124.9 million samples/s (median of 6 runs). 1.01x the previous value.
